# ChunLI-666/PointCloudProcessor

Hardware: AMD Instinct MI355X
Metric: Mpoints×frames/sec colorized (higher is better)
Workload: dtype f32/f64

## Files before the change

### include/pcp_hip.h

```cpp
#ifndef PCP_HIP_H
#define PCP_HIP_H

#include <stdint.h>

#ifdef __cplusplus
extern "C" {
#endif

#define PCP_ABI_VERSION 6

#define PCP_OK 0
#define PCP_ERR_INVALID (-1)
#define PCP_ERR_STATE (-2)
#define PCP_ERR_DEVICE (-3)
#define PCP_ERR_NOMEM (-4)
#define PCP_ERR_RANGE (-5)

typedef struct pcp_context pcp_context;

typedef struct pcp_pose {
  double x, y, z, qw, qx, qy, qz;
} pcp_pose;

typedef struct pcp_camera {
// ... 202 lines not shown
#define PCP_ASCII_PARSE_MAX_ROW 65536
#define PCP_PARSE_LIMIT_ROW 0
#define PCP_PARSE_LIMIT_TILE 1
#define PCP_PARSE_LIMIT_PIECE 2
#define PCP_PARSE_LIMIT_TILE_ROWS 3
#define PCP_PARSE_LIMIT_WINDOW 4
int64_t pcp_ascii_parse_limit(int32_t which);
int pcp_ascii_parse_host(const char *text, int64_t bytes, int32_t columns, const int32_t col[4], int32_t final_window,
                         int64_t max_rows, float *out_x, float *out_y, float *out_z, float *out_intensity,
                         int64_t *out_rows, int64_t *out_consumed, int64_t *out_bad_row);
int pcp_ascii_parse(pcp_context *ctx, const char *text, int64_t bytes, int32_t columns, const int32_t col[4], int32_t final_window,
                    int64_t max_rows, float *out_x, float *out_y, float *out_z, float *out_intensity,
                    int64_t *out_rows, int64_t *out_consumed, int64_t *out_bad_row);

int pcp_voxel_reduce_begin(pcp_context *ctx, float leaf, int64_t initial_slots);
int pcp_voxel_reduce_add(pcp_context *ctx, int64_t *out_rows_added);
int pcp_voxel_reduce_finish(pcp_context *ctx, int64_t *out_voxels);
int pcp_voxel_reduce_fetch(pcp_context *ctx, int64_t first, int64_t max_rows, float *out_xyz, uint8_t *out_rgb, uint8_t *out_label,
                           uint32_t *out_count, int64_t *out_rows);
int pcp_voxel_reduce_stats(pcp_context *ctx, int64_t out[6]);
int pcp_voxel_reduce_end(pcp_context *ctx);
int pcp_voxel_reduce_host(float leaf, int64_t n, const float *xyz, const uint8_t *rgb, const uint8_t *label, int64_t capacity,
                          float *out_xyz, uint8_t *out_rgb, uint8_t *out_label, uint32_t *out_count, int64_t *out_voxels);

typedef struct pcp_ortho_frame {
  float o[3], u[3], v[3], n[3];
  float gsd;
  int32_t width, height;
  float d_min, d_max;
} pcp_ortho_frame;
int pcp_ortho_begin(pcp_context *ctx, const pcp_ortho_frame *frame);
int pcp_ortho_add(pcp_context *ctx, int64_t index_base, int64_t *out_contributors);
int pcp_ortho_add_packed(pcp_context *ctx, const uint32_t *rgba, int64_t index_base, int64_t *out_contributors);
int pcp_ortho_finish(pcp_context *ctx, int32_t fill_radius_px, int64_t *out_occupied, int64_t *out_filled);
int pcp_ortho_fetch(pcp_context *ctx, uint32_t *out_index, float *out_depth, uint8_t *out_rgb, uint8_t *out_label,
                    uint8_t *out_status, int32_t *out_source);
int pcp_ortho_stats(pcp_context *ctx, int64_t out[6]);
int pcp_ortho_end(pcp_context *ctx);
int pcp_ortho_host(const pcp_ortho_frame *frame, int64_t n, const float *xyz, const uint8_t *rgb, const uint8_t *label,
                   const uint8_t *has, int64_t index_base, int32_t fill_radius_px, uint32_t *out_index, float *out_depth,
                   uint8_t *out_rgb, uint8_t *out_label, uint8_t *out_status, int32_t *out_source, int64_t *out_contributors,
                   int64_t *out_occupied, int64_t *out_filled);
int pcp_ortho_fit_frame_host(int64_t n, const float *xyz, const uint8_t *has, const double *viewer, float gsd, pcp_ortho_frame *out);

typedef struct pcp_ortho_texture_params {
  int32_t scale;
  int32_t x0, y0, w, h;
  int32_t views;
  int32_t interpolate;
  float max_step;
} pcp_ortho_texture_params;
int pcp_ortho_texture(pcp_context *ctx, const pcp_ortho_texture_params *params, uint8_t *out_rgb, uint8_t *out_mask,
                      uint8_t *out_status, int16_t *out_view, uint8_t *out_count, int64_t out_counts[4]);
int pcp_ortho_texture_points_host(const pcp_ortho_frame *frame, const pcp_ortho_texture_params *params, const int32_t *source,
                                  const float *depth, float *out_xyz, uint8_t *out_ok);

#define PCP_BALANCE_CLAHE 1
#define PCP_BALANCE_GAMMA 2
typedef struct pcp_balance_params {
  int32_t stages;
  int32_t tiles_x, tiles_y;
  float clip_limit;
  float gamma;
} pcp_balance_params;
void pcp_default_balance_params(pcp_balance_params *p);
int pcp_set_image_balance(pcp_context *ctx, const pcp_balance_params *params);
int pcp_image_balance_host(const pcp_balance_params *params, int32_t w, int32_t h, const uint8_t *bgr, int64_t row_stride_bytes,
                           uint8_t *out_bgr, uint32_t *out_hist, uint8_t *out_lut);
int pcp_image_balance(pcp_context *ctx, const pcp_balance_params *params, int32_t w, int32_t h, const uint8_t *bgr,
                      int64_t row_stride_bytes, uint8_t *out_bgr, uint32_t *out_hist, uint8_t *out_lut);
int pcp_gamma_table_host(float gamma, uint8_t out[256]);

int pcp_estimate_normals(pcp_context *ctx, float radius, int64_t *out_valid, int64_t *out_moments);
int pcp_normals_fetch(pcp_context *ctx, float *out_normal, float *out_curvature, int32_t *out_neighbours);
int pcp_normals_moments_host(float radius, int64_t n, const float *xyz, int64_t *out_moments);
int pcp_frame_geometry(pcp_context *ctx, int32_t frame, int32_t *out_index, float *out_range, float *out_xyz_cam,
                       float *out_normal_cam, int64_t *out_pixels);

int pcp_mask_edt(pcp_context *ctx, int32_t frame, int32_t threshold, uint32_t *out_d2, int32_t *out_nearest);
int pcp_mask_edt_frames(pcp_context *ctx, int32_t first_frame, int32_t count, int32_t threshold, uint32_t *out_d2,
                        int32_t *out_nearest);
int pcp_mask_edt_host(int32_t width, int32_t height, const uint8_t *gray, int64_t row_stride_bytes, int32_t threshold,
                      uint32_t *out_d2, int32_t *out_nearest);

typedef struct pcp_crack_params {
  int32_t threshold;
  int32_t plane_radius_px;
} pcp_crack_params;
int pcp_crack_width(pcp_context *ctx, int32_t frame, const pcp_crack_params *params, uint8_t *out_flags, int32_t *out_edges,
                    uint32_t *out_w2d2, float *out_width, float *out_points, float *out_plane, int64_t *out_moments,
                    int64_t *out_sites, int64_t *out_widths);
int pcp_crack_width_host(int32_t width, int32_t height, const uint8_t *gray, int64_t row_stride_bytes, const int32_t *index_image,
                         const float *xyz_cam_image, const pcp_crack_params *params, uint8_t *out_flags, int32_t *out_edges,
                         uint32_t *out_w2d2, int64_t *out_moments);

typedef struct pcp_crack_link_params {
  int32_t min_views;
  float radius;
} pcp_crack_link_params;
int pcp_crack_fuse_begin(pcp_context *ctx);
int pcp_crack_fuse_add(pcp_context *ctx, int32_t frame, const pcp_crack_params *params, int64_t *out_contributors,
                       int64_t *out_credited);
int pcp_crack_fuse_fetch(pcp_context *ctx, float *out_width_mean, float *out_width_best, int32_t *out_best_frame, uint32_t *out_views,
                         uint32_t *out_seen, uint32_t *out_centres, uint32_t *out_min_q, uint32_t *out_max_q, uint64_t *out_sum_q);
int pcp_crack_fuse_end(pcp_context *ctx);
int pcp_crack_fuse_host(int64_t n, uint32_t *seen, uint32_t *views, uint32_t *centres, uint32_t *min_q, uint32_t *max_q,
                        uint32_t *best_q, uint64_t *sum_q, uint64_t *best_key, int64_t m, const int32_t *index, const int32_t *pixel,
                        const float *range, int32_t frame, int32_t width, int32_t height, const uint8_t *flags, const float *width_image,
                        int64_t *out_credited);
int pcp_crack_components(pcp_context *ctx, const pcp_crack_link_params *p, int32_t *out_label, int64_t *out_crack_points,
                         int64_t *out_components);
int pcp_crack_components_fetch(pcp_context *ctx, int64_t first, int64_t max_rows, int32_t *out_id, int64_t *out_stats, float *out_box,
                               int64_t *out_rows);
int pcp_crack_components_host(int64_t n, const float *xyz, const uint32_t *views, int32_t min_views, float radius, int32_t *out_label,
                              int64_t *out_components);

int pcp_crack_lengths(pcp_context *ctx, const pcp_crack_link_params *p, uint64_t *out_pos, int64_t *out_cracks, int64_t *out_path_points);
int pcp_crack_lengths_fetch(pcp_context *ctx, int64_t first, int64_t max_rows, int32_t *out_id, int64_t *out_rows7, int64_t *out_offsets,
                            int64_t *out_rows);
int pcp_crack_paths_fetch(pcp_context *ctx, int64_t first_entry, int64_t max_entries, int32_t *out_index, int64_t *out_entries);
int pcp_crack_lengths_host(int64_t n, const float *xyz, const uint32_t *views, int32_t min_views, float radius, const uint64_t *sum_q,
                           uint64_t *out_pos, int32_t *out_id, int64_t *out_rows7, int64_t *out_offsets, int32_t *out_path,
                           int64_t *out_cracks, int64_t *out_path_points);

int pcp_crack_skeleton(pcp_context *ctx, const pcp_crack_link_params *p, float step, int32_t *out_node, int64_t *out_nodes, int64_t *out_edges);
int pcp_crack_skeleton_nodes_fetch(pcp_context *ctx, int64_t first, int64_t max_rows, int32_t *out_id, int64_t *out_rows10, int64_t *out_rows);
int pcp_crack_skeleton_edges_fetch(pcp_context *ctx, int64_t first, int64_t max_rows, int64_t *out_rows3, int64_t *out_rows);
int pcp_crack_skeleton_cracks_fetch(pcp_context *ctx, int64_t first, int64_t max_rows, int64_t *out_rows6, int64_t *out_rows);
int pcp_crack_skeleton_host(int64_t n, const float *xyz, const uint32_t *views, int32_t min_views, float radius, float step,
                            const uint64_t *sum_q, int32_t *out_node, int32_t *out_id, int64_t *out_rows10, int64_t edge_capacity,
                            int64_t *out_rows3, int64_t *out_rows6, int64_t *out_nodes, int64_t *out_edges, int64_t *out_cracks);

typedef struct pcp_facet_params {
  float link_radius, angle_deg, plane_tol, max_curvature;
  int32_t min_points;
} pcp_facet_params;
int pcp_facets(pcp_context *ctx, const pcp_facet_params *params, int32_t *out_label, int64_t *out_facet_points, int64_t *out_components,
               int64_t *out_facets);
int pcp_facets_fetch(pcp_context *ctx, int64_t first, int64_t max_rows, int32_t *out_id, int64_t *out_rows10, float *out_box,
                     int64_t *out_rows);
int pcp_facets_host(int64_t n, const float *xyz, const float *normal, const float *curvature, const pcp_facet_params *params,
                    int32_t *out_label, int32_t *out_id, int64_t *out_rows10, float *out_box, int64_t *out_facets);
int pcp_facet_plane_host(const float root[3], const int64_t row10[10], double out_plane[7]);
int pcp_ortho_add_facet(pcp_context *ctx, int32_t facet_id, int64_t index_base, int64_t *out_contributors);

int pcp_close_pairs(pcp_context *ctx, double radius, int64_t *points_with_close_neighbour);

int pcp_timing_enable(pcp_context *ctx, int32_t on);
int pcp_timing_reset(pcp_context *ctx);
int pcp_timing_get(pcp_context *ctx, int32_t kernel_id, double *total_ms, int64_t *launches);
const char *pcp_kernel_name(int32_t kernel_id);
int pcp_tile_mask_density(pcp_context *ctx, double *kept_fraction);
int pcp_tile_masks(pcp_context *ctx, int64_t *tiles, int32_t *mask_words, uint32_t *out_words);
int pcp_sor_redo_fraction(pcp_context *ctx, double *fraction);
int pcp_sor_distances(pcp_context *ctx, int64_t capacity, float *out_distance);
int pcp_selftest_arithmetic(pcp_context *ctx, int64_t samples, uint64_t seed, int64_t *mismatches_fp64,
                            int64_t *mismatches_fp32);
int pcp_selftest_visit_forms(pcp_context *ctx, int64_t samples, uint64_t seed, int64_t *mismatches_uv, int64_t *mismatches_cell,
                             int64_t *mismatches_sqrt, int32_t *short_distortion);
int pcp_selftest_k3_term(pcp_context *ctx, int64_t samples, uint64_t seed, int64_t *mismatches, int32_t *term_dropped);

#ifdef __cplusplus
}
#endif
#endif
```

### pointcloudprocessor_amd/_build.py

```python
from __future__ import annotations

import os
import subprocess

_PKG = os.path.dirname(os.path.abspath(__file__))
_ROOT = os.path.dirname(_PKG)
CSRC = os.path.join(_PKG, "csrc")
LIB_DIR = os.path.join(_PKG, "lib")
LIB_PATH = os.path.join(LIB_DIR, "libpcp_hip.so")
INCLUDE = os.path.join(_ROOT, "include")

SOURCES = ["pcp_context.hip", "pcp_colour.hip", "pcp_mls.hip", "pcp_grid.hip", "pcp_nid.hip", "pcp_hpr.hip", "pcp_colour_smooth.hip", "pcp_match.hip", "pcp_jpeg.hip",
           "pcp_stream_colour.hip", "pcp_ascii.hip", "pcp_ascii_parse.hip", "pcp_exposure.hip", "pcp_voxel_reduce.hip", "pcp_normals.hip", "pcp_mask_edt.hip", "pcp_ortho.hip", "pcp_ortho_texture.hip", "pcp_facets.hip", "pcp_crack_width.hip", "pcp_crack_fuse.hip", "pcp_crack_length.hip", "pcp_crack_skeleton.hip", "pcp_image_balance.hip"]
HEADERS = ["pcp_internal.hpp", "pcp_device.hpp", "pcp_scan.hpp", "pcp_hsv.hpp", "pcp_exact.hpp", "pcp_ascii.hpp", "pcp_ascii_parse.hpp", "pcp_visit_forms.hpp", "pcp_voxel_reduce.hpp", "pcp_eigen33.hpp", "pcp_eigen33_host.hpp", "pcp_facets.hpp", "pcp_normals.hpp", "pcp_mask_edt.hpp", "pcp_ortho.hpp", "pcp_ortho_texture.hpp", "pcp_tile_classify.hpp", "pcp_crack_width.hpp", "pcp_crack_fuse.hpp", "pcp_crack_length.hpp", "pcp_crack_skeleton.hpp", "pcp_crack_map.hpp", "pcp_image_balance.hpp"]

HIPCC_FLAGS = [
    "--offload-arch=gfx950",
    "-O3",
    "-std=c++17",
    "-fPIC",
    "-ffp-contract=off",
    "-fhip-fp32-correctly-rounded-divide-sqrt",
    "-Wall",
    "-Wextra",
]


def _hipcc() -> str:
    for cand in (os.environ.get("HIPCC"), "/opt/rocm/bin/hipcc", "hipcc"):
        if cand and (os.path.isabs(cand) and os.path.exists(cand) or not os.path.isabs(cand)):
            return cand
    return "hipcc"


def source_sha256() -> str:
    import hashlib

    h = hashlib.sha256()
    h.update(" ".join(HIPCC_FLAGS).encode())
    for f in [os.path.join(CSRC, f) for f in SOURCES + HEADERS] + [os.path.join(INCLUDE, "pcp_hip.h")]:
        h.update(os.path.basename(f).encode())
        with open(f, "rb") as fh:
            h.update(fh.read())
    return h.hexdigest()


def is_stale() -> bool:
    if not os.path.exists(LIB_PATH):
        return True
    t = os.path.getmtime(LIB_PATH)
    deps = [os.path.join(CSRC, f) for f in SOURCES + HEADERS] + [os.path.join(INCLUDE, "pcp_hip.h")]
    return any(os.path.getmtime(d) > t for d in deps)


def build(force: bool = False, verbose: bool = False) -> str:
    if not force and not is_stale():
        return LIB_PATH
    os.makedirs(LIB_DIR, exist_ok=True)
    from concurrent.futures import ThreadPoolExecutor

    obj_dir = os.path.join(LIB_DIR, "obj")
    os.makedirs(obj_dir, exist_ok=True)
    inc = ["-I", os.path.relpath(INCLUDE, CSRC), "-I", "."]

    def compile_one(src):
        stem = os.path.splitext(src)[0]
        obj = os.path.join(os.path.relpath(obj_dir, CSRC), stem + ".o")
        cmd = [_hipcc()] + HIPCC_FLAGS + inc + [f"-cuid={stem}", "-c", src, "-o", obj]
        return cmd, subprocess.run(cmd, capture_output=True, text=True, cwd=CSRC)

    with ThreadPoolExecutor(max_workers=len(SOURCES)) as pool:
        results = list(pool.map(compile_one, SOURCES))
    log = ""
    for cmd, proc in results:
        if verbose or proc.returncode != 0:
            log += " ".join(cmd) + "\n" + proc.stdout + proc.stderr
    if any(proc.returncode != 0 for _, proc in results):
        print(log)
        raise RuntimeError("hipcc failed building libpcp_hip.so:\n" + log[-4000:])
    objs = [os.path.join(os.path.relpath(obj_dir, CSRC), os.path.splitext(src)[0] + ".o") for src in SOURCES]
    link = [_hipcc(), "--offload-arch=gfx950", "--hip-link", "-shared", "-fPIC", "-o", LIB_PATH] + objs
    proc = subprocess.run(link, capture_output=True, text=True, cwd=CSRC)
    if verbose or proc.returncode != 0:
        print(log + " ".join(link))
        print(proc.stdout)
        print(proc.stderr)
    if proc.returncode != 0:
        raise RuntimeError("hipcc failed linking libpcp_hip.so:\n" + proc.stderr[-4000:])
    return LIB_PATH


if __name__ == "__main__":
    print(build(force=True, verbose=True))
```

### pointcloudprocessor_amd/capi.py

```python
from __future__ import annotations

import ctypes as C
import os
import re

import numpy as np

from . import _build

PCP_OK = 0
PCP_ERR_INVALID = -1
PCP_ERR_STATE = -2
PCP_ERR_DEVICE = -3
PCP_ERR_NOMEM = -4
PCP_ERR_RANGE = -5

NID_EVAL_FN = C.CFUNCTYPE(C.c_int, C.c_void_p, C.POINTER(C.c_double), C.c_int32, C.POINTER(C.c_double), C.POINTER(C.c_double),
                          C.POINTER(C.c_int32))
K_PROJECT, K_DEPTH, K_COLOUR, K_VISIBILITY, K_MLS_GRID, K_MLS_FIT, K_MISC, K_SOR, K_MLS_VOXEL, K_TILE_MASK, K_NID, K_HPR = range(12)
K_COLOUR_SMOOTH = 12
K_COUNT = 13


class PcpError(RuntimeError):
# ... 1394 lines not shown
    def sor(self, mean_k: int = 60, std_mul: float = 0.7):
        keep = np.empty(self.n, np.uint8)
        kept = C.c_int64()
        self._check(self.lib.pcp_sor(self.h, C.c_int32(mean_k), C.c_double(std_mul), _ptr(keep), C.byref(kept)))
        return keep, kept.value

    def sor_chunk_points(self) -> int:
        return int(self.lib.pcp_sor_chunk_points())

    def sor_partial(self, mean_k: int, slab: int, n_slabs: int):
        c = self.sor_chunk_points()
        chunks = (self.n + c - 1) // c
        out = np.zeros((max(chunks, 1), 2), np.float64)
        first, cnt = C.c_int64(), C.c_int64()
        self._check(self.lib.pcp_sor_partial(self.h, C.c_int32(mean_k), C.c_int32(slab), C.c_int32(n_slabs), C.c_int64(len(out)),
                                             _ptr(out), C.byref(first), C.byref(cnt)))
        return first.value, out[:cnt.value].copy()

    def sor_finish(self, std_mul: float, all_chunk_sums: np.ndarray, slab: int, n_slabs: int):
        sums = np.ascontiguousarray(all_chunk_sums, np.float64)
        keep = np.empty(self.n, np.uint8)
        kept = C.c_int64()
        self._check(self.lib.pcp_sor_finish(self.h, C.c_double(std_mul), _ptr(sums), C.c_int64(len(sums)), C.c_int32(slab),
                                            C.c_int32(n_slabs), _ptr(keep), C.byref(kept)))
        return keep, kept.value

    def close_pairs(self, radius: float = 2.5e-5) -> int:
        cnt = C.c_int64()
        self._check(self.lib.pcp_close_pairs(self.h, C.c_double(radius), C.byref(cnt)))
        return cnt.value

    def sor_distances(self) -> np.ndarray:
        out = np.empty(self.n, np.float32)
        self._check(self.lib.pcp_sor_distances(self.h, C.c_int64(len(out)), _ptr(out)))
        return out

    def sor_redo_fraction(self) -> float:
        v = C.c_double()
        self._check(self.lib.pcp_sor_redo_fraction(self.h, C.byref(v)))
        return v.value

    def upload_intensity(self, intensity):
        a = np.ascontiguousarray(intensity, np.float32)
        self._check(self.lib.pcp_upload_intensity(self.h, _ptr(a), C.c_int64(len(a))))

    def nid_prepare(self) -> int:
        cnt = C.c_int64()
        self._check(self.lib.pcp_nid_prepare(self.h, C.byref(cnt)))
        return cnt.value

    def nid_evaluate(self, T, T_init=None, bins: int = 16):
        T = np.ascontiguousarray(T, np.float64).reshape(16)
        Ti = None if T_init is None else np.ascontiguousarray(T_init, np.float64).reshape(16)
        cost = C.c_double()
        grad = np.zeros(6, np.float64)
        valid = C.c_int32()
        self._check(self.lib.pcp_nid_evaluate(self.h, _ptr(T), _ptr(Ti), C.c_int32(bins), C.byref(cost), _ptr(grad),
                                              C.byref(valid)))
        return cost.value, grad, bool(valid.value)

    def nid_optimize(self, T_init, bins: int = 16, max_outer_iterations: int = 10):
        Ti = np.ascontiguousarray(T_init, np.float64).reshape(16)
        out = np.zeros(16, np.float64)
        cost = C.c_double()
        evals = C.c_int32()
        self._check(self.lib.pcp_nid_optimize(self.h, _ptr(Ti), C.c_int32(bins), C.c_int32(max_outer_iterations), _ptr(out),
                                              C.byref(cost), C.byref(evals)))
        return out.reshape(4, 4), cost.value, evals.value

    def nid_accumulate(self, T, bins: int = 16):
        T = np.ascontiguousarray(T, np.float64).reshape(16)
        self._check(self.lib.pcp_nid_accumulate(self.h, _ptr(T), C.c_int32(bins)))

    def nid_histograms_device(self):
        p = C.c_void_p()
        n = C.c_int64()
        self._check(self.lib.pcp_nid_histograms_device(self.h, C.byref(p), C.byref(n)))
        return p.value, n.value

    def nid_finish(self, bins: int = 16):
        cost = C.c_double()
        grad = np.zeros(6, np.float64)
        valid = C.c_int32()
        self._check(self.lib.pcp_nid_finish(self.h, C.c_int32(bins), C.byref(cost), _ptr(grad), C.byref(valid)))
        return cost.value, grad, bool(valid.value)

    def nid_optimize_with(self, evaluate, T_init, bins: int = 16, max_outer_iterations: int = 10):
        errors = []

        @NID_EVAL_FN
        def trampoline(_user, T, b, cost, grad, valid):
            try:
                c, g, ok = evaluate(np.ctypeslib.as_array(T, (16,)).copy().reshape(4, 4), int(b))
                cost[0] = float(c)
                for k in range(6):
                    grad[k] = float(g[k])
                valid[0] = 1 if ok else 0
                return 0
            except Exception as e:
                errors.append(e)
                return -3

        Ti = np.ascontiguousarray(T_init, np.float64).reshape(16)
        out = np.zeros(16, np.float64)
        cost = C.c_double()
        evals = C.c_int32()
        rc = self.lib.pcp_nid_optimize_with(self.h, trampoline, None, _ptr(Ti), C.c_int32(bins), C.c_int32(max_outer_iterations),
                                            _ptr(out), C.byref(cost), C.byref(evals))
        if errors:
            raise errors[0]
        self._check(rc)
        return out.reshape(4, 4), cost.value, evals.value

    def timing_enable(self, on: bool = True):
        self._check(self.lib.pcp_timing_enable(self.h, C.c_int32(1 if on else 0)))

    def timing_reset(self):
        self._check(self.lib.pcp_timing_reset(self.h))

    def timing_get(self, kernel_id: int):
        ms = C.c_double()
        cnt = C.c_int64()
        self._check(self.lib.pcp_timing_get(self.h, C.c_int32(kernel_id), C.byref(ms), C.byref(cnt)))
        return ms.value, cnt.value

    def tile_mask_density(self) -> float:
        v = C.c_double()
        self._check(self.lib.pcp_tile_mask_density(self.h, C.byref(v)))
        return v.value

    def selftest_arithmetic(self, samples: int = 1 << 26, seed: int = 1):
        a, b = C.c_int64(), C.c_int64()
        self._check(self.lib.pcp_selftest_arithmetic(self.h, C.c_int64(samples), C.c_uint64(seed), C.byref(a), C.byref(b)))
        return a.value, b.value

    def selftest_visit_forms(self, samples: int = 1 << 24, seed: int = 1):
        a, b, c, f = C.c_int64(), C.c_int64(), C.c_int64(), C.c_int32()
        self._check(self.lib.pcp_selftest_visit_forms(self.h, C.c_int64(samples), C.c_uint64(seed), C.byref(a), C.byref(b), C.byref(c),
                                                      C.byref(f)))
        return a.value, b.value, c.value, bool(f.value)

    def selftest_k3_term(self, samples: int = 1 << 24, seed: int = 1):
        a, f = C.c_int64(), C.c_int32()
        self._check(self.lib.pcp_selftest_k3_term(self.h, C.c_int64(samples), C.c_uint64(seed), C.byref(a), C.byref(f)))
        return a.value, bool(f.value)

    def tile_masks(self) -> np.ndarray:
        t, w = C.c_int64(), C.c_int32()
        self._check(self.lib.pcp_tile_masks(self.h, C.byref(t), C.byref(w), None))
        out = np.empty((t.value, w.value), np.uint32)
        self._check(self.lib.pcp_tile_masks(self.h, None, None, _ptr(out)))
        return out

    def kernel_name(self, kernel_id: int) -> str:
        return self.lib.pcp_kernel_name(C.c_int32(kernel_id)).decode()
```

### pointcloudprocessor_amd/csrc/pcp_colour.hip

```cpp
#include <algorithm>
#include <cfloat>
#include <cstdlib>

#include "pcp_device.hpp"
#include "pcp_hsv.hpp"
#include "pcp_scan.hpp"
#include "pcp_tile_classify.hpp"

namespace pcp {

constexpr int kBlock = 256;
constexpr uint32_t kFltMaxBits = 0x7f7fffffu;

template <bool kCommon>
__device__ __forceinline__ DevCamera common_camera(const DevCamera &in) {
  DevCamera c = in;
  if constexpr (kCommon) {
    c.cull_mode = PCP_CULL_ZBUFFER;
    c.enable_zbuf = 1;
    c.pretest = 1;
    c.ds_fast = 1;
  }
  return c;
}
inline bool is_common_camera(const pcp_context *ctx) {
  const DevCamera &c = ctx->dcam;
  return c.cull_mode == PCP_CULL_ZBUFFER && c.enable_zbuf == 1 && c.pretest == 1 && c.ds_fast == 1 && ctx->uv_tame;
}

struct ProjectOut {
  int32_t *cell;
  int32_t *pixel;
  float *range;
  float *xc, *yc, *zc;
};

__device__ __forceinline__ void project_store_one(const DevCamera &cam, const DevFrame &fr, float x, float y, float z,
                                                  int32_t &cell, int32_t &pixel, float &range, float &xc, float &yc,
                                                  float &zc) {
  const Projected p = project_point<true, false>(cam, fr.w2c, x, y, z);
  cell = p.cell;
  pixel = p.pixel;
  range = p.cell != -1 ? static_cast<float>(range64(p.xc, p.yc, p.zc)) : FLT_MAX;
  xc = p.xc;
  yc = p.yc;
  zc = p.zc;
}

template <bool kCommon>
__global__ __launch_bounds__(kBlock) void k_project_frame(const float *__restrict__ x, const float *__restrict__ y,
                                                          const float *__restrict__ z, int64_t n, DevCamera cam_in,
                                                          DevFrame fr, ProjectOut out) {
  const DevCamera cam = common_camera<kCommon>(cam_in);
  const int64_t q = static_cast<int64_t>(blockIdx.x) * kBlock + threadIdx.x;
  const int64_t i0 = q * 4;
  if (i0 >= n) return;
  if (i0 + 3 < n) {
    typedef float nt_f4 __attribute__((ext_vector_type(4)));
    typedef int nt_i4 __attribute__((ext_vector_type(4)));
    const nt_f4 ax = __builtin_nontemporal_load(reinterpret_cast<const nt_f4 *>(x + i0));
    const nt_f4 ay = __builtin_nontemporal_load(reinterpret_cast<const nt_f4 *>(y + i0));
    const nt_f4 az = __builtin_nontemporal_load(reinterpret_cast<const nt_f4 *>(z + i0));
    const float4 vx = make_float4(ax.x, ax.y, ax.z, ax.w), vy = make_float4(ay.x, ay.y, ay.z, ay.w),
                 vz = make_float4(az.x, az.y, az.z, az.w);
    int4 cell, pixel;
    float4 range, xc, yc, zc;
    project_store_one(cam, fr, vx.x, vy.x, vz.x, cell.x, pixel.x, range.x, xc.x, yc.x, zc.x);
    project_store_one(cam, fr, vx.y, vy.y, vz.y, cell.y, pixel.y, range.y, xc.y, yc.y, zc.y);
    project_store_one(cam, fr, vx.z, vy.z, vz.z, cell.z, pixel.z, range.z, xc.z, yc.z, zc.z);
    project_store_one(cam, fr, vx.w, vy.w, vz.w, cell.w, pixel.w, range.w, xc.w, yc.w, zc.w);
    if (out.cell) {
      const nt_i4 c4 = {cell.x, cell.y, cell.z, cell.w};
      __builtin_nontemporal_store(c4, reinterpret_cast<nt_i4 *>(out.cell + i0));
    }
    if (out.range) {
      const nt_f4 r4 = {range.x, range.y, range.z, range.w};
      __builtin_nontemporal_store(r4, reinterpret_cast<nt_f4 *>(out.range + i0));
    }
    if (out.pixel) *reinterpret_cast<int4 *>(out.pixel + i0) = pixel;
    if (out.xc) {
      *reinterpret_cast<float4 *>(out.xc + i0) = xc;
      *reinterpret_cast<float4 *>(out.yc + i0) = yc;
      *reinterpret_cast<float4 *>(out.zc + i0) = zc;
    }
  } else {
    for (int64_t i = i0; i < n; ++i) {
      int32_t cell, pixel;
      float range, xc, yc, zc;
      project_store_one(cam, fr, x[i], y[i], z[i], cell, pixel, range, xc, yc, zc);
      if (out.cell) out.cell[i] = cell;
      if (out.range) out.range[i] = range;
      if (out.pixel) out.pixel[i] = pixel;
      if (out.xc) {
        out.xc[i] = xc;
        out.yc[i] = yc;
        out.zc[i] = zc;
      }
    }
  }
}

constexpr int kTileGroup = 16;

__global__ __launch_bounds__(kBlock) void k_group_mask_flat(const float4 *__restrict__ spheres, int64_t groups, DevCamera cam,
                                                            const DevFrame *__restrict__ frames, int32_t n_frames,
                                                            int32_t w0, int32_t w1, int32_t words,
                                                            uint32_t *__restrict__ group_mask,
                                                            uint32_t *__restrict__ group_inside, int32_t cull_enabled,
                                                            int32_t *__restrict__ zeroed, int32_t n_zeroed,
                                                            unsigned long long *__restrict__ far_maps, int64_t far_cells) {
  const int64_t idx = static_cast<int64_t>(blockIdx.x) * kBlock + threadIdx.x;
  if (idx < n_zeroed) zeroed[idx] = 0;
  for (int64_t c = idx; c < far_cells; c += static_cast<int64_t>(gridDim.x) * kBlock) far_maps[c] = 0x7f7f7f7f7f7f7f7full;
  const int32_t nw = w1 - w0;
  const int64_t gw = idx >> 5;
  const int64_t group = gw / nw;
  const bool live = group < groups;
  const int32_t w = w0 + static_cast<int32_t>(gw - group * nw);
  const int32_t f = (w << 5) + static_cast<int32_t>(idx & 31);
  int cls = 1;
  if (live && f < n_frames) cls = cull_enabled ? tile_classify(cam, frames[f], spheres[group]) : 0;
  const unsigned long long m = __ballot(cls != 1), in = __ballot(cls == 2);
  if (live && (idx & 31) == 0) {
    group_mask[group * words + w] = static_cast<uint32_t>((threadIdx.x & 32) ? (m >> 32) : m);
    group_inside[group * words + w] = static_cast<uint32_t>((threadIdx.x & 32) ? (in >> 32) : in);
  }
}

template <bool kInside>
__global__ __launch_bounds__(kBlock) void k_tile_mask_dense(const float4 *__restrict__ spheres, int64_t tiles,
                                                            DevCamera cam, const DevFrame *__restrict__ frames,
                                                            int32_t n_frames, int32_t w0, int32_t w1, int32_t words,
                                                            const uint32_t *__restrict__ group_mask,
                                                            const uint32_t *__restrict__ group_inside,
                                                            uint32_t *__restrict__ tile_mask,
                                                            uint32_t *__restrict__ inside_mask, int32_t cull_enabled) {
  const int lane = threadIdx.x & 63;
  const int32_t nw = w1 - w0;
  const int64_t gw = static_cast<int64_t>(blockIdx.x) * (kBlock / 64) + (threadIdx.x >> 6);
  const int64_t group = gw / nw;
  if (group >= (tiles + kTileGroup - 1) / kTileGroup) return;
  const int32_t w = w0 + static_cast<int32_t>(gw - group * nw);
  const int t = lane & 15, slot = lane >> 4;
  const int64_t tile = group * kTileGroup + t;
  const bool have = tile < tiles;
  uint32_t todo = __builtin_amdgcn_readfirstlane(group_mask[group * words + w]);
  const int32_t nb = n_frames - (w << 5);
  if (nb < 32) todo &= nb <= 0 ? 0u : ((1u << nb) - 1u);
  const uint32_t whole = __builtin_amdgcn_readfirstlane(group_inside[group * words + w]) & todo;
  todo &= ~whole;
  uint32_t word = whole;
  [[maybe_unused]] uint32_t inside = whole;
  if (todo) {
    const float4 sph = spheres[have ? tile : tiles - 1];
    while (todo) {
      int32_t bit[4];
#pragma unroll
      for (int k = 0; k < 4; ++k) {
        bit[k] = todo ? __builtin_ctz(todo) : -1;
        todo &= todo - (todo ? 1u : 0u);
      }
      const int32_t b = slot == 0 ? bit[0] : slot == 1 ? bit[1] : slot == 2 ? bit[2] : bit[3];
      int cls = 1;
      if (b >= 0 && have) cls = cull_enabled ? tile_classify(cam, frames[(w << 5) + b], sph) : 0;
      const unsigned long long keep = __ballot(cls != 1);
      [[maybe_unused]] unsigned long long ins = 0ull;
      if constexpr (kInside) ins = __ballot(cls == 2);
#pragma unroll
      for (int k = 0; k < 4; ++k) {
        if (bit[k] >= 0) {
          word |= static_cast<uint32_t>((keep >> (k * 16 + t)) & 1ull) << bit[k];
          if constexpr (kInside) inside |= static_cast<uint32_t>((ins >> (k * 16 + t)) & 1ull) << bit[k];
        }
      }
    }
  }
  if (slot == 0 && have) {
    tile_mask[tile * words + w] = word;
    if constexpr (kInside) {
      if (inside_mask) inside_mask[tile * words + w] = inside;
    }
  }
}

constexpr int kWorkBins = 1024;
constexpr int kWorkPerBlock = 1024;
__global__ __launch_bounds__(kBlock) void k_tile_work_hist(const uint32_t *__restrict__ tile_mask, int64_t tiles, int32_t w0,
                                                          int32_t w1, int32_t words, int32_t *__restrict__ tile_work,
                                                          int32_t *__restrict__ hist) {
  __shared__ int32_t cnt[kWorkBins];
  for (int b = threadIdx.x; b < kWorkBins; b += kBlock) cnt[b] = 0;
  __syncthreads();
  const int64_t base = static_cast<int64_t>(blockIdx.x) * kWorkPerBlock;
  for (int q = 0; q < kWorkPerBlock / kBlock; ++q) {
    const int64_t t = base + q * kBlock + threadIdx.x;
    if (t < tiles) {
      int32_t visits = 0;
      for (int32_t w = w0; w < w1; ++w) visits += __builtin_popcount(tile_mask[t * words + w]);
      tile_work[t] = visits;
      atomicAdd(&cnt[min(visits, kWorkBins - 1)], 1);
    }
  }
  __syncthreads();
  for (int b = threadIdx.x; b < kWorkBins; b += kBlock)
    if (cnt[b]) atomicAdd(&hist[b], cnt[b]);
}
__global__ __launch_bounds__(kBlock) void k_work_scatter(const int32_t *__restrict__ work, int64_t tiles,
                                                        const int32_t *__restrict__ hist, int32_t *__restrict__ cursor,
                                                        int32_t *__restrict__ order) {
  __shared__ int32_t cnt[kWorkBins];
  __shared__ int32_t first[kWorkBins];
  __shared__ int32_t ws[kScanBlock / 64];
  for (int b = threadIdx.x; b < kWorkBins; b += kBlock) cnt[b] = 0;
  {
    constexpr int kPer = kWorkBins / kBlock;
    int32_t h[kPer], mine = 0;
#pragma unroll
    for (int k = 0; k < kPer; ++k) {
      h[k] = hist[kWorkBins - 1 - (static_cast<int>(threadIdx.x) * kPer + k)];
      mine += h[k];
    }
    int32_t total = 0;
    int32_t run = scan_block_exclusive(mine, &total, ws);
#pragma unroll
    for (int k = 0; k < kPer; ++k) {
      first[kWorkBins - 1 - (static_cast<int>(threadIdx.x) * kPer + k)] = run;
      run += h[k];
    }
  }
  __syncthreads();
  const int64_t base = static_cast<int64_t>(blockIdx.x) * kWorkPerBlock;
  int32_t bin[kWorkPerBlock / kBlock], rank[kWorkPerBlock / kBlock];
#pragma unroll
  for (int q = 0; q < kWorkPerBlock / kBlock; ++q) {
    const int64_t t = base + q * kBlock + threadIdx.x;
    bin[q] = t < tiles ? min(work[t], kWorkBins - 1) : -1;
    rank[q] = bin[q] >= 0 ? atomicAdd(&cnt[bin[q]], 1) : 0;
  }
  __syncthreads();
  for (int b = threadIdx.x; b < kWorkBins; b += kBlock)
    if (cnt[b]) cnt[b] = first[b] + atomicAdd(&cursor[b], cnt[b]);
  __syncthreads();
#pragma unroll
  for (int q = 0; q < kWorkPerBlock / kBlock; ++q)
    if (bin[q] >= 0) order[cnt[bin[q]] + rank[q]] = static_cast<int32_t>(base + q * kBlock + threadIdx.x);
}

constexpr uint32_t kXcdChunk = 16;
__device__ __forceinline__ uint32_t xcd_chunked_block() {
  constexpr uint32_t kXcd = 8, kSuper = kXcd * kXcdChunk;
  const uint32_t b = blockIdx.x;
  if (b >= (gridDim.x / kSuper) * kSuper) return b;
  const uint32_t x = b % kXcd, slot = b / kXcd;
  return ((slot / kXcdChunk) * kXcd + x) * kXcdChunk + slot % kXcdChunk;
}

constexpr unsigned long long kDepthEmpty = 0x7f7f7f7f7f7f7f7full;
__device__ __forceinline__ void depth_min(unsigned long long *__restrict__ map, int32_t cell, unsigned long long bits) {
  if (bits < map[cell]) atomicMin(map + cell, bits);
}
__device__ __forceinline__ double sumsq64(float xc, float yc, float zc) {
  const double X = xc, Y = yc, Z = zc;
  return (X * X + Y * Y) + Z * Z;
}
__global__ __launch_bounds__(kBlock) void k_depth_finish(const unsigned long long *__restrict__ sq, int64_t count,
                                                         uint32_t *__restrict__ range) {
  int64_t i = static_cast<int64_t>(blockIdx.x) * kBlock + threadIdx.x;
  const int64_t stride = static_cast<int64_t>(gridDim.x) * kBlock;
  for (; i < count; i += stride) {
    const unsigned long long b = sq[i];
    float r = FLT_MAX;
    if (b != kDepthEmpty) r = fminf(static_cast<float>(sqrt(__longlong_as_double(static_cast<long long>(b)))), FLT_MAX);
    range[i] = __float_as_uint(r);
  }
}

__device__ __forceinline__ uint32_t range_bits(int32_t w, int32_t f0, int32_t f1) {
  const int32_t fb = max(f0, w << 5), fe = min(f1, (w << 5) + 32);
  const int32_t nb = fe - fb;
  return nb <= 0 ? 0u : (((nb >= 32) ? 0xffffffffu : ((1u << nb) - 1u)) << (fb & 31));
}

template <bool kCommon, bool kK3 = true>
__global__ __launch_bounds__(kBlock) void k_depth_pass(const float *__restrict__ x, const float *__restrict__ y,
                                                       const float *__restrict__ z, int64_t n, DevCamera cam_in,
                                                       const DevFrame *__restrict__ frames, int32_t f0, int32_t f1,
                                                       unsigned long long *__restrict__ depth, int64_t cells,
                                                       int32_t depth_first_frame, uint32_t *__restrict__ tile_mask,
                                                       const uint32_t *__restrict__ tile_inside, int32_t words,
                                                       const int32_t *__restrict__ tile_order) {
  DevCamera cam = common_camera<kCommon>(cam_in);
  if constexpr (kCommon) cam.pretest = 0;
  __shared__ unsigned long long combine[kBlock];
  const int lane = threadIdx.x & 63;
  unsigned long long *tbl = combine + (threadIdx.x & ~63);
  const int64_t j = tile_order ? static_cast<int64_t>(tile_order[blockIdx.x]) * 64 + threadIdx.x
                               : static_cast<int64_t>(xcd_chunked_block()) * kBlock + threadIdx.x;
  const bool live = j < n;
  if (!__ballot(live)) return;
  const float px = live ? x[j] : 0.0f, py = live ? y[j] : 0.0f, pz = live ? z[j] : 0.0f;
  const int64_t tile = __builtin_amdgcn_readfirstlane(static_cast<int32_t>(j >> 6));
  const bool finite_sure = cam.frames_bounded != 0 && __all(fabsf(px) <= 0x1p40f && fabsf(py) <= 0x1p40f && fabsf(pz) <= 0x1p40f);
  unsigned long long *held_at = nullptr;
  unsigned long long held_bits = 0ull, held_seen = 0ull;
  auto settle_held = [&]() {
    if (held_at && held_bits < held_seen) atomicMin(held_at, held_bits);
    held_at = nullptr;
  };
  const int32_t w_last = (f1 - 1) >> 5;
  for (int32_t wbase = f0 >> 5; wbase <= w_last; wbase += 64) {
    const int32_t my_w = wbase + lane;
    const bool have_w = my_w <= w_last;
    uint32_t my_word = 0xffffffffu;
    if (tile_mask && have_w) my_word = tile_mask[tile * words + my_w];
    [[maybe_unused]] uint32_t my_inside = 0u;
    if constexpr (!kCommon) {
      if (tile_inside && have_w) my_inside = tile_inside[tile * words + my_w];
// ... 1277 lines not shown

int pcp_project_frame(pcp_context *ctx, int32_t frame, int32_t *out_cell, int32_t *out_pixel, float *out_range,
                      float *out_xyz_cam) {
  int rc = check_ready(ctx, "pcp_project_frame", true);
  if (rc != PCP_OK) return rc;
  if ((rc = check_frame(ctx, "pcp_project_frame", frame)) != PCP_OK) return rc;
  const int64_t n = ctx->n;
  const size_t plane = plane_of(ctx);
  PCP_HIP_TRY(ctx, ctx->s_cell.ensure(plane + 4));
  PCP_HIP_TRY(ctx, ctx->s_range.ensure(plane + 4));
  if (out_pixel) PCP_HIP_TRY(ctx, ctx->s_pixel.ensure(plane + 4));
  if (out_xyz_cam) PCP_HIP_TRY(ctx, ctx->s_cam.ensure(3 * plane + 4));
  if (n == 0) return PCP_OK;
  ProjectOut o{};
  o.cell = ctx->s_cell.p;
  o.range = ctx->s_range.p;
  o.pixel = out_pixel ? ctx->s_pixel.p : nullptr;
  o.xc = out_xyz_cam ? ctx->s_cam.p : nullptr;
  o.yc = out_xyz_cam ? ctx->s_cam.p + plane : nullptr;
  o.zc = out_xyz_cam ? ctx->s_cam.p + 2 * plane : nullptr;
  {
    LaunchTimer t(ctx, PCP_K_PROJECT);
    hipLaunchKernelGGL(is_common_camera(ctx) ? k_project_frame<true> : k_project_frame<false>, dim3(blocks_for(div_up(n, 4))), dim3(kBlock), 0, ctx->stream, ctx->sxyz.p,
                       ctx->sxyz.p + plane, ctx->sxyz.p + 2 * plane, n, ctx->dcam,
                       ctx->hframes[static_cast<size_t>(frame)], o);
    PCP_HIP_TRY(ctx, hipGetLastError());
  }
  if (!(out_cell || out_range || out_pixel || out_xyz_cam)) return PCP_OK;
  const size_t sn = static_cast<size_t>(n);
  PCP_HIP_TRY(ctx, ctx->s_u32.ensure(plane + 4));
  auto fetch = [&](const void *sorted, void *host) -> int {
    {
      LaunchTimer t(ctx, PCP_K_MISC);
      hipLaunchKernelGGL(k_scatter_u32, dim3(blocks_for(n)), dim3(kBlock), 0, ctx->stream,
                         static_cast<const uint32_t *>(sorted), ctx->perm.p, n, ctx->s_u32.p);
      PCP_HIP_TRY(ctx, hipGetLastError());
    }
    PCP_HIP_TRY(ctx, hipMemcpyAsync(host, ctx->s_u32.p, sn * 4, hipMemcpyDeviceToHost, ctx->stream));
    PCP_HIP_TRY(ctx, hipStreamSynchronize(ctx->stream));
    return PCP_OK;
  };
  if (out_cell && (rc = fetch(o.cell, out_cell)) != PCP_OK) return rc;
  if (out_range && (rc = fetch(o.range, out_range)) != PCP_OK) return rc;
  if (out_pixel && (rc = fetch(o.pixel, out_pixel)) != PCP_OK) return rc;
  if (out_xyz_cam) {
    if ((rc = fetch(o.xc, out_xyz_cam)) != PCP_OK) return rc;
    if ((rc = fetch(o.yc, out_xyz_cam + sn)) != PCP_OK) return rc;
    if ((rc = fetch(o.zc, out_xyz_cam + 2 * sn)) != PCP_OK) return rc;
  }
  return PCP_OK;
}

int pcp_cull_frame(pcp_context *ctx, int32_t frame, uint8_t *out_keep, int64_t *out_kept, float *out_depth_map) {
  int rc = check_ready(ctx, "pcp_cull_frame", true);
  if (rc != PCP_OK) return rc;
  if ((rc = check_frame(ctx, "pcp_cull_frame", frame)) != PCP_OK) return rc;
  const int64_t n = ctx->n;
  if ((rc = single_frame_depth(ctx, frame)) != PCP_OK) return rc;
  if ((rc = frame_keep_flags(ctx, frame, false)) != PCP_OK) return rc;
  if (out_kept) {
    int64_t cnt = 0;
    if (n > 0 && (rc = compact_flags(ctx, ctx->s_keep.p, n, nullptr, 0, &cnt)) != PCP_OK) return rc;
    *out_kept = cnt;
  }
  if (out_keep && n > 0)
    PCP_HIP_TRY(ctx, hipMemcpyAsync(out_keep, ctx->s_keep.p, static_cast<size_t>(n), hipMemcpyDefault, ctx->stream));
  if (out_depth_map)
    PCP_HIP_TRY(ctx, hipMemcpyAsync(out_depth_map, ctx->s_u32.p, static_cast<size_t>(cells_of(ctx)) * 4,
                                    hipMemcpyDeviceToHost, ctx->stream));
  PCP_HIP_TRY(ctx, hipStreamSynchronize(ctx->stream));
  return PCP_OK;
}

int pcp_frame_visible(pcp_context *ctx, int32_t frame, int64_t capacity, int32_t *out_index, uint8_t *out_rgb,
                      uint16_t *out_mask, float *out_xyz_cam, float *out_xyz_world, int64_t *out_count) {
  int rc = check_ready(ctx, "pcp_frame_visible", true);
  if (rc != PCP_OK) return rc;
  if ((rc = check_frame(ctx, "pcp_frame_visible", frame)) != PCP_OK) return rc;
  if (capacity < 0) return set_error(ctx, PCP_ERR_INVALID, "pcp_frame_visible: negative capacity");
  const int64_t n = ctx->n;
  if (out_count) *out_count = 0;
  if (n == 0) return PCP_OK;
  if ((rc = ensure_images(ctx)) != PCP_OK) return rc;
  if ((rc = wait_images(ctx, frame, frame + 1)) != PCP_OK) return rc;
  int64_t m = 0;
  if ((rc = visible_indices(ctx, frame, &m)) != PCP_OK) return rc;
  const size_t plane = plane_of(ctx);
  if (out_count) *out_count = m;
  const int64_t take = std::min(m, capacity);
  if (take == 0) return PCP_OK;
  const size_t st = static_cast<size_t>(take);
  PCP_HIP_TRY(ctx, ctx->s_range.ensure(st + 4));
  const bool want_cam = out_xyz_cam != nullptr, want_world = out_xyz_world != nullptr;
  PCP_HIP_TRY(ctx, ctx->s_cam.ensure((want_cam ? 3 * st : 0) + (want_world ? 3 * st : 0) + 4));
  float *d_cam = want_cam ? ctx->s_cam.p : nullptr;
  float *d_world = want_world ? ctx->s_cam.p + (want_cam ? 3 * st : 0) : nullptr;
  const int64_t px = static_cast<int64_t>(ctx->dcam.img_w) * ctx->dcam.img_h;
  {
    LaunchTimer t(ctx, PCP_K_MISC);
    hipLaunchKernelGGL(k_gather_visible, dim3(blocks_for(take)), dim3(kBlock), 0, ctx->stream, ctx->xyz.p,
                       ctx->xyz.p + plane, ctx->xyz.p + 2 * plane, ctx->dcam, ctx->hframes[static_cast<size_t>(frame)],
                       ctx->s_cell.p, take, ctx->images.p + static_cast<int64_t>(frame) * px,
                       static_cast<int32_t>(ctx->image_set[static_cast<size_t>(frame)]),
                       static_cast<int32_t>(ctx->mask_set[static_cast<size_t>(frame)]),
                       reinterpret_cast<uint32_t *>(ctx->s_range.p), d_cam, d_world);
    PCP_HIP_TRY(ctx, hipGetLastError());
  }
  std::vector<uint32_t> rgbm;
  if (out_rgb || out_mask) {
    rgbm.resize(st);
    PCP_HIP_TRY(ctx, hipMemcpyAsync(rgbm.data(), ctx->s_range.p, st * 4, hipMemcpyDeviceToHost, ctx->stream));
  }
  if (out_index) PCP_HIP_TRY(ctx, hipMemcpyAsync(out_index, ctx->s_cell.p, st * 4, hipMemcpyDeviceToHost, ctx->stream));
  if (want_cam) PCP_HIP_TRY(ctx, hipMemcpyAsync(out_xyz_cam, d_cam, 3 * st * 4, hipMemcpyDeviceToHost, ctx->stream));
  if (want_world) PCP_HIP_TRY(ctx, hipMemcpyAsync(out_xyz_world, d_world, 3 * st * 4, hipMemcpyDeviceToHost, ctx->stream));
  PCP_HIP_TRY(ctx, hipStreamSynchronize(ctx->stream));
  for (size_t k = 0; k < rgbm.size(); ++k) {
    if (out_rgb) {
      out_rgb[3 * k + 0] = static_cast<uint8_t>(rgbm[k] & 0xffu);
      out_rgb[3 * k + 1] = static_cast<uint8_t>((rgbm[k] >> 8) & 0xffu);
      out_rgb[3 * k + 2] = static_cast<uint8_t>((rgbm[k] >> 16) & 0xffu);
    }
    if (out_mask) out_mask[k] = static_cast<uint16_t>(rgbm[k] >> 24);
  }
  return PCP_OK;
}

int pcp_depth_pass(pcp_context *ctx, int32_t frame_begin, int32_t frame_end) {
  int rc = check_ready(ctx, "pcp_depth_pass", true);
  if (rc != PCP_OK) return rc;
  if (frame_begin < 0 || frame_end > ctx->n_frames || frame_begin > frame_end)
    return set_error(ctx, PCP_ERR_RANGE, "pcp_depth_pass: keyframe range [%d,%d) outside 0..%d", frame_begin, frame_end,
                     ctx->n_frames);
  if (frame_begin == frame_end) return PCP_OK;
  if ((rc = ensure_depth(ctx)) != PCP_OK) return rc;
  const int64_t cells = cells_of(ctx);
  const int64_t map_cells = static_cast<int64_t>(frame_end - frame_begin) * cells;
  const bool z_maps = ctx->n > 0 && ctx->dcam.enable_zbuf;
  if (z_maps) {
    PCP_HIP_TRY(ctx, ctx->depth_sq.ensure(static_cast<size_t>(map_cells) + 4));
  } else if ((rc = fill_u32(ctx, ctx->depth.p + static_cast<int64_t>(frame_begin) * cells, map_cells, kFltMaxBits)) != PCP_OK) {
    return rc;
  }
  if (ctx->n > 0) {
    const size_t plane = plane_of(ctx);
    const int32_t w0 = frame_begin >> 5, w1 = ((frame_end - 1) >> 5) + 1;
    static const bool cull_tiles = [] {
      const char *e = std::getenv("PCP_DISABLE_TILE_CULL");
      return !(e && e[0] == '1');
    }();
    {
      LaunchTimer t(ctx, PCP_K_TILE_MASK);
      const int64_t groups = div_up(ctx->n_tiles, kTileGroup);
      const float4 *tile_sph = reinterpret_cast<const float4 *>(ctx->tile_sphere.p);
      const size_t gwords = static_cast<size_t>(groups) * ctx->mask_words;
      PCP_HIP_TRY(ctx, ctx->group_mask.ensure(2 * gwords + 8));
      uint32_t *group_inside = ctx->group_mask.p + gwords + 4;
      hipLaunchKernelGGL(k_group_mask_flat, dim3(std::max(blocks_for(groups * (w1 - w0) * 32), blocks_for(2 * kWorkBins))),
                         dim3(kBlock), 0, ctx->stream, tile_sph + ctx->n_tiles, groups, ctx->dcam, ctx->frames.p, ctx->n_frames,
                         w0, w1, ctx->mask_words, ctx->group_mask.p, group_inside, cull_tiles ? 1 : 0, ctx->work_hist.p,
                         2 * kWorkBins, z_maps ? reinterpret_cast<unsigned long long *>(ctx->depth_sq.p) : nullptr,
                         z_maps ? map_cells : int64_t(0));
      uint32_t *tile_inside = is_common_camera(ctx) ? nullptr : ctx->tile_inside.p;
      hipLaunchKernelGGL(tile_inside ? k_tile_mask_dense<true> : k_tile_mask_dense<false>, dim3(static_cast<uint32_t>(div_up(groups * (w1 - w0), kBlock / 64))), dim3(kBlock),
                         0, ctx->stream, tile_sph, ctx->n_tiles, ctx->dcam, ctx->frames.p, ctx->n_frames, w0, w1,
                         ctx->mask_words, ctx->group_mask.p, group_inside, ctx->tile_mask.p, tile_inside, cull_tiles ? 1 : 0);
      if ((rc = sort_tiles_by_work(ctx, w0, w1, ctx->tile_order.p)) != PCP_OK) return rc;
      ctx->tile_order_live = true;
    }
    if (ctx->cull.cull_mode == PCP_CULL_HPR) {
      int rch = ensure_hull_bits(ctx);
      if (rch != PCP_OK) return rch;
      if (!ctx->depth_from_batch) {
        int32_t clear_until = frame_begin;
        for (int32_t f = frame_begin; f < frame_end; ++f) {
          uint32_t *hull_plane = ctx->hull_bits.p + static_cast<size_t>(f >> 5) * static_cast<size_t>(ctx->n);
          if ((f & 31) == 0 && std::min(f + 32, ctx->n_frames) <= frame_end) {
            PCP_HIP_TRY(ctx, hipMemsetAsync(hull_plane, 0, static_cast<size_t>(ctx->n) * 4, ctx->stream));
            clear_until = std::min(f + 32, ctx->n_frames);
          }
          if (f >= clear_until) {
            LaunchTimer t(ctx, PCP_K_HPR);
            hipLaunchKernelGGL(k_hull_clear, dim3(blocks_for(ctx->n)), dim3(kBlock), 0, ctx->stream, hull_plane, ctx->n, 1u << (f & 31));
          }
        }
        PCP_HIP_TRY(ctx, hipGetLastError());
        const char *le = std::getenv("PCP_HPR_LANES");
        const int32_t lanes = le && le[0] >= '1' && le[0] <= '8' ? le[0] - '0' : 4;
        if ((rc = hpr_run_range(ctx, frame_begin, frame_end, lanes, ctx->tile_mask.p)) != PCP_OK) return rc;
        for (int32_t f = frame_begin; f < frame_end; ++f) ctx->hull_valid[static_cast<size_t>(f)] = 1;
      }
    }
    {
      LaunchTimer t(ctx, PCP_K_DEPTH);
      const bool common = is_common_camera(ctx);
      auto kernel = !common ? k_depth_pass<false> : ctx->k3_dropped ? k_depth_pass<true, false> : k_depth_pass<true>;
      hipLaunchKernelGGL(kernel,
                         dim3(static_cast<uint32_t>(ctx->n_tiles)), dim3(64), 0, ctx->stream, ctx->sxyz.p,
                         ctx->sxyz.p + plane, ctx->sxyz.p + 2 * plane, ctx->n, ctx->dcam, ctx->frames.p, frame_begin,
                         frame_end, ctx->depth_sq.p, cells, frame_begin, ctx->tile_mask.p,
                         common ? static_cast<const uint32_t *>(nullptr) : ctx->tile_inside.p, ctx->mask_words, ctx->tile_order.p);
      if (z_maps)
        hipLaunchKernelGGL(k_depth_finish, dim3(static_cast<uint32_t>(std::min<int64_t>(div_up(map_cells, kBlock), 4096))),
                           dim3(kBlock), 0, ctx->stream, ctx->depth_sq.p, map_cells,
                           ctx->depth.p + static_cast<int64_t>(frame_begin) * cells);
      PCP_HIP_TRY(ctx, hipGetLastError());
    }
  }
  for (int32_t f = frame_begin; f < frame_end; ++f) ctx->depth_valid[static_cast<size_t>(f)] = 1;
  return PCP_OK;
}

int pcp_depth_maps_device(pcp_context *ctx, void **device_ptr, int64_t *n_floats) {
  int rc = check_ready(ctx, "pcp_depth_maps_device", true);
  if (rc != PCP_OK) return rc;
  if (ctx->cull.cull_mode == PCP_CULL_HPR)
    return set_error(ctx, PCP_ERR_STATE, "pcp_depth_maps_device: PCP_CULL_HPR has no depth maps to merge across point shards "
                     "(the hull needs the whole map on one GPU)");
  if ((rc = ensure_depth(ctx)) != PCP_OK) return rc;
  if (device_ptr) *device_ptr = ctx->depth.p;
  if (n_floats) *n_floats = cells_of(ctx) * ctx->n_frames;
  return PCP_OK;
}

int pcp_set_depth_source(pcp_context *ctx, int32_t source) {
  if (!ctx) return PCP_ERR_INVALID;
  if (source != PCP_DEPTH_OWN && source != PCP_DEPTH_BATCHED)
    return set_error(ctx, PCP_ERR_INVALID, "pcp_set_depth_source: unknown source %d", source);
  ctx->depth_from_batch = source == PCP_DEPTH_BATCHED;
  return PCP_OK;
}

int pcp_hull_flags_import(pcp_context *ctx, int32_t frame, const uint8_t *keep) {
  int rc = check_ready(ctx, "pcp_hull_flags_import", true);
  if (rc != PCP_OK) return rc;
  if ((rc = check_frame(ctx, "pcp_hull_flags_import", frame)) != PCP_OK) return rc;
  if (ctx->cull.cull_mode != PCP_CULL_HPR || !ctx->depth_from_batch)
    return set_error(ctx, PCP_ERR_STATE, "pcp_hull_flags_import: needs cull_mode PCP_CULL_HPR and pcp_set_depth_source(PCP_DEPTH_BATCHED)");
  if (!keep && ctx->n > 0) return set_error(ctx, PCP_ERR_INVALID, "pcp_hull_flags_import: NULL flags");
  if ((rc = ensure_hull_bits(ctx)) != PCP_OK) return rc;
  if (ctx->n > 0) {
    PCP_HIP_TRY(ctx, ctx->s_keep.ensure(static_cast<size_t>(ctx->n) + 16));
    PCP_HIP_TRY(ctx, hipMemcpyAsync(ctx->s_keep.p, keep, static_cast<size_t>(ctx->n), hipMemcpyDefault, ctx->stream));
    if ((rc = store_hull_bits(ctx, frame, false)) != PCP_OK) return rc;
    PCP_HIP_TRY(ctx, hipStreamSynchronize(ctx->stream));
  }
  ctx->hull_valid[static_cast<size_t>(frame)] = 1;
  return PCP_OK;
}

int pcp_download_depth_map(pcp_context *ctx, int32_t frame, float *out_depth_map) {
  int rc = check_ready(ctx, "pcp_download_depth_map", true);
  if (rc != PCP_OK) return rc;
  if ((rc = check_frame(ctx, "pcp_download_depth_map", frame)) != PCP_OK) return rc;
  if (!out_depth_map) return set_error(ctx, PCP_ERR_INVALID, "pcp_download_depth_map: NULL output");
  if (!ctx->depth.p || !ctx->depth_valid[static_cast<size_t>(frame)])
    return set_error(ctx, PCP_ERR_STATE, "pcp_download_depth_map: pcp_depth_pass has not covered keyframe %d", frame);
  const int64_t cells = cells_of(ctx);
  PCP_HIP_TRY(ctx, hipMemcpyAsync(out_depth_map, ctx->depth.p + static_cast<int64_t>(frame) * cells,
                                  static_cast<size_t>(cells) * 4, hipMemcpyDeviceToHost, ctx->stream));
  PCP_HIP_TRY(ctx, hipStreamSynchronize(ctx->stream));
  return PCP_OK;
}

int pcp_colour_reset(pcp_context *ctx) {
  if (!ctx) return PCP_ERR_INVALID;
  ctx->colour_state_live = false;
  ctx->colour_result_live = false;
  ctx->labels_live = false;
  return PCP_OK;
}

static int begin_result(pcp_context *ctx, uint32_t **dst) {
  const int32_t cur = ctx->rgba_cur ^ 1;
  PCP_HIP_TRY(ctx, ctx->rgba2[cur].ensure(static_cast<size_t>(ctx->n) + 4));
  if (ctx->copy_pending[cur]) {
    PCP_HIP_TRY(ctx, hipStreamWaitEvent(ctx->stream, ctx->copy_done[cur], 0));
    ctx->copy_pending[cur] = false;
  }
  *dst = ctx->rgba2[cur].p;
  return PCP_OK;
}

static int labels_begin(pcp_context *ctx) {
  ctx->labels_live = false;
  if (!ctx->label_fusion) return PCP_OK;
  PCP_HIP_TRY(ctx, ctx->labels.ensure(static_cast<size_t>(ctx->n) + 4));
  PCP_HIP_TRY(ctx, hipMemsetAsync(ctx->labels.p + ctx->n, 0, 4, ctx->stream));
  return PCP_OK;
}

static int labels_end(pcp_context *ctx) {
  if (!ctx->label_fusion) return PCP_OK;
  uint32_t bad = 0;
  uint32_t *dst = ctx->readback ? static_cast<uint32_t *>(ctx->readback) : &bad;
  PCP_HIP_TRY(ctx, hipMemcpyAsync(dst, ctx->labels.p + ctx->n, 4, hipMemcpyDeviceToHost, ctx->stream));
  PCP_HIP_TRY(ctx, hipStreamSynchronize(ctx->stream));
  if (*dst != 0)
    return set_error(ctx, PCP_ERR_RANGE, "label fusion: a view score outside [2^-3, 2) reached the label arithmetic "
                     "(final_score cannot produce one): no labels for this result");
  ctx->labels_live = true;
  return PCP_OK;
}

static int check_masks(pcp_context *ctx, int32_t frame_begin, int32_t frame_end) {
  if (!ctx->label_fusion) return PCP_OK;
  for (int32_t f = frame_begin; f < frame_end; ++f)
    if (static_cast<size_t>(f) >= ctx->mask_set.size() || !ctx->mask_set[static_cast<size_t>(f)])
      return set_error(ctx, PCP_ERR_STATE, "pcp_colour_pass: label fusion is on and no mask was uploaded for keyframe %d", f);
  return PCP_OK;
}

static int colour_pass_impl(pcp_context *ctx, int32_t frame_begin, int32_t frame_end, bool one_shot,
                            uint32_t *result = nullptr) {
  int rc = check_ready(ctx, "pcp_colour_pass", true);
  if (rc != PCP_OK) return rc;
  if (frame_begin < 0 || frame_end > ctx->n_frames || frame_begin > frame_end)
    return set_error(ctx, PCP_ERR_RANGE, "pcp_colour_pass: keyframe range [%d,%d) outside 0..%d", frame_begin, frame_end,
// ... 123 lines not shown
    if ((rc = finalise_gained(ctx, result)) != PCP_OK) return rc;
  } else if (n > 0) {
    TopState st{ctx->top_score.p, ctx->top_rgb.p, ctx->top_frame.p, ctx->view_count.p};
    LaunchTimer t(ctx, PCP_K_COLOUR);
    const bool label = ctx->label_fusion;
    const LabelOut lab{label ? ctx->labels.p : nullptr};
    if (label)
      hipLaunchKernelGGL(k_finalise_labels, dim3(blocks_for(n)), dim3(kBlock), 0, ctx->stream, n, st, ctx->perm.p, result, lab);
    else
      hipLaunchKernelGGL(k_finalise, dim3(blocks_for(n)), dim3(kBlock), 0, ctx->stream, n, st, ctx->perm.p, result);
    PCP_HIP_TRY(ctx, hipGetLastError());
  }
  if ((rc = labels_end(ctx)) != PCP_OK) return rc;
  if ((rc = end_result(ctx, out_rgb, out_has)) != PCP_OK) return rc;
  if ((out_count || out_top_score || out_top_rgb || out_top_frame) && n > 0) {
    std::vector<int32_t> perm(sn), cnt;
    std::vector<uint32_t> tmp(kTopM * sn);
    PCP_HIP_TRY(ctx, hipMemcpyAsync(perm.data(), ctx->perm.p, sn * 4, hipMemcpyDeviceToHost, ctx->stream));
    auto fetch5 = [&](const void *src, void *dst_v) -> int {
      PCP_HIP_TRY(ctx, hipMemcpyAsync(tmp.data(), src, kTopM * sn * 4, hipMemcpyDeviceToHost, ctx->stream));
      PCP_HIP_TRY(ctx, hipStreamSynchronize(ctx->stream));
      uint32_t *dst = static_cast<uint32_t *>(dst_v);
      for (size_t j = 0; j < sn; ++j)
        for (int k = 0; k < kTopM; ++k) dst[static_cast<size_t>(perm[j]) * kTopM + k] = tmp[static_cast<size_t>(k) * sn + j];
      return PCP_OK;
    };
    if (out_top_score && (rc = fetch5(ctx->top_score.p, out_top_score)) != PCP_OK) return rc;
    if (out_top_rgb && (rc = fetch5(ctx->top_rgb.p, out_top_rgb)) != PCP_OK) return rc;
    if (out_top_rgb && ctx->label_fusion)
      for (size_t k = 0; k < kTopM * sn; ++k) out_top_rgb[k] &= 0xffffffu;
    if (out_top_frame && (rc = fetch5(ctx->top_frame.p, out_top_frame)) != PCP_OK) return rc;
    if (out_count) {
      cnt.resize(sn);
      PCP_HIP_TRY(ctx, hipMemcpyAsync(cnt.data(), ctx->view_count.p, sn * 4, hipMemcpyDeviceToHost, ctx->stream));
      PCP_HIP_TRY(ctx, hipStreamSynchronize(ctx->stream));
      for (size_t j = 0; j < sn; ++j) out_count[perm[j]] = cnt[j];
    }
  }
  return PCP_OK;
}

static int refuse_gains(pcp_context *ctx, const char *who) {
  if (!ctx->gains_set) return PCP_OK;
  return set_error(ctx, PCP_ERR_STATE, "%s: exposure gains are set (pcp_set_frame_gains): they apply to pcp_colour_reset / "
                   "pcp_colour_pass / pcp_colour_finalise; clear them with pcp_set_frame_gains(NULL) for the one-shot call", who);
}

int pcp_colorize(pcp_context *ctx, uint8_t *out_rgb, uint8_t *out_has) {
  int rc = check_ready(ctx, "pcp_colorize", true);
  if (rc != PCP_OK) return rc;
  if ((rc = refuse_gains(ctx, "pcp_colorize")) != PCP_OK) return rc;
  if ((rc = check_masks(ctx, 0, ctx->n_frames)) != PCP_OK) return rc;
  pcp_colour_reset(ctx);
  if ((rc = pcp_depth_pass(ctx, 0, ctx->n_frames)) != PCP_OK) return rc;
  uint32_t *result = nullptr;
  if ((rc = begin_result(ctx, &result)) != PCP_OK) return rc;
  if ((rc = labels_begin(ctx)) != PCP_OK) return rc;
  if ((rc = colour_pass_impl(ctx, 0, ctx->n_frames, true, result)) != PCP_OK) return rc;
  if ((rc = labels_end(ctx)) != PCP_OK) return rc;
  return end_result(ctx, out_rgb, out_has);
}

int pcp_colorize_from_depth(pcp_context *ctx, uint8_t *out_rgb, uint8_t *out_has) {
  int rc = check_ready(ctx, "pcp_colorize_from_depth", true);
  if (rc != PCP_OK) return rc;
  if ((rc = refuse_gains(ctx, "pcp_colorize_from_depth")) != PCP_OK) return rc;
  pcp_colour_reset(ctx);
  uint32_t *result = nullptr;
  if ((rc = begin_result(ctx, &result)) != PCP_OK) return rc;
  if ((rc = labels_begin(ctx)) != PCP_OK) return rc;
  if ((rc = colour_pass_impl(ctx, 0, ctx->n_frames, true, result)) != PCP_OK) return rc;
  if ((rc = labels_end(ctx)) != PCP_OK) return rc;
  return end_result(ctx, out_rgb, out_has);
}

int pcp_colour_smooth_local(pcp_context *ctx, float radius, int64_t *out_has_count) {
  if (!ctx) return PCP_ERR_INVALID;
  if (!smooth_radius_ok(radius))
    return set_error(ctx, PCP_ERR_INVALID, "pcp_colour_smooth_local: radius %g outside (0, 1]", static_cast<double>(radius));
  if (!ctx->colour_result_live)
    return set_error(ctx, PCP_ERR_STATE, "pcp_colour_smooth_local: no result (call pcp_colorize / pcp_colour_finalise)");
  if (out_has_count) *out_has_count = 0;
  if (ctx->n == 0) return PCP_OK;
  PCP_HIP_TRY(ctx, hipSetDevice(ctx->device));
  const uint32_t *src = ctx->rgba2[ctx->rgba_cur].p;
  uint32_t *dst = nullptr;
  int rc = begin_result(ctx, &dst);
  if (rc != PCP_OK) return rc;
  if ((rc = colour_smooth_words(ctx, radius, src, dst, out_has_count)) != PCP_OK) return rc;
  return end_result(ctx, nullptr, nullptr);
}

int pcp_download_result_packed(pcp_context *ctx, uint32_t *out_rgba) {
  if (!ctx) return PCP_ERR_INVALID;
  if (!ctx->colour_result_live)
    return set_error(ctx, PCP_ERR_STATE, "pcp_download_result_packed: no result (call pcp_colorize / pcp_colour_finalise)");
  if (!out_rgba && ctx->n > 0) return set_error(ctx, PCP_ERR_INVALID, "pcp_download_result_packed: NULL output");
  if (ctx->n > 0)
    PCP_HIP_TRY(ctx, hipMemcpyAsync(out_rgba, ctx->rgba2[ctx->rgba_cur].p, static_cast<size_t>(ctx->n) * 4,
                                    hipMemcpyDeviceToHost, ctx->stream));
  PCP_HIP_TRY(ctx, hipStreamSynchronize(ctx->stream));
  return PCP_OK;
}

int pcp_download_result_packed_async(pcp_context *ctx, uint32_t *out_rgba) {
  if (!ctx) return PCP_ERR_INVALID;
  if (!ctx->colour_result_live)
    return set_error(ctx, PCP_ERR_STATE, "pcp_download_result_packed_async: no result (call pcp_colorize / pcp_colour_finalise)");
  if (!out_rgba && ctx->n > 0) return set_error(ctx, PCP_ERR_INVALID, "pcp_download_result_packed_async: NULL output");
  const int32_t cur = ctx->rgba_cur;
  PCP_HIP_TRY(ctx, hipStreamWaitEvent(ctx->copy_stream, ctx->result_ready[cur], 0));
  if (ctx->n > 0)
    PCP_HIP_TRY(ctx, hipMemcpyAsync(out_rgba, ctx->rgba2[cur].p, static_cast<size_t>(ctx->n) * 4, hipMemcpyDeviceToHost,
                                    ctx->copy_stream));
  PCP_HIP_TRY(ctx, hipEventRecord(ctx->copy_done[cur], ctx->copy_stream));
  ctx->copy_pending[cur] = true;
  return PCP_OK;
}

int pcp_download_wait_previous(pcp_context *ctx) {
  if (!ctx) return PCP_ERR_INVALID;
  const int32_t prev = ctx->rgba_cur ^ 1;
  if (ctx->copy_pending[prev]) PCP_HIP_TRY(ctx, hipEventSynchronize(ctx->copy_done[prev]));
  return PCP_OK;
}

int pcp_tile_mask_density(pcp_context *ctx, double *kept_fraction) {
  if (!ctx || !kept_fraction) return PCP_ERR_INVALID;
  if (!ctx->tile_mask.p || ctx->n_tiles == 0 || ctx->n_frames == 0)
    return set_error(ctx, PCP_ERR_STATE, "pcp_tile_mask_density: no masks (call pcp_depth_pass)");
  std::vector<uint32_t> h(static_cast<size_t>(ctx->n_tiles) * ctx->mask_words);
  PCP_HIP_TRY(ctx, hipMemcpyAsync(h.data(), ctx->tile_mask.p, h.size() * 4, hipMemcpyDeviceToHost, ctx->stream));
  PCP_HIP_TRY(ctx, hipStreamSynchronize(ctx->stream));
  uint64_t bits = 0;
  for (uint32_t w : h) bits += static_cast<uint64_t>(__builtin_popcount(w));
  *kept_fraction = static_cast<double>(bits) / (static_cast<double>(ctx->n_tiles) * ctx->n_frames);
  return PCP_OK;
}

int pcp_tile_masks(pcp_context *ctx, int64_t *tiles, int32_t *mask_words, uint32_t *out_words) {
  if (!ctx) return PCP_ERR_INVALID;
  if (!ctx->tile_mask.p || ctx->n_tiles == 0 || ctx->n_frames == 0)
    return set_error(ctx, PCP_ERR_STATE, "pcp_tile_masks: no masks (call pcp_depth_pass)");
  if (tiles) *tiles = ctx->n_tiles;
  if (mask_words) *mask_words = ctx->mask_words;
  if (out_words) {
    PCP_HIP_TRY(ctx, hipMemcpyAsync(out_words, ctx->tile_mask.p, static_cast<size_t>(ctx->n_tiles) * ctx->mask_words * 4,
                                    hipMemcpyDeviceToHost, ctx->stream));
    PCP_HIP_TRY(ctx, hipStreamSynchronize(ctx->stream));
  }
  return PCP_OK;
}

int pcp_colour_result_device(pcp_context *ctx, void **device_ptr, int64_t *n_words) {
  if (!ctx) return PCP_ERR_INVALID;
  if (!ctx->colour_result_live)
    return set_error(ctx, PCP_ERR_STATE, "pcp_colour_result_device: no result (call pcp_colorize / pcp_colour_finalise)");
  if (device_ptr) *device_ptr = ctx->rgba2[ctx->rgba_cur].p;
  if (n_words) *n_words = ctx->n;
  return PCP_OK;
}

int pcp_set_label_fusion(pcp_context *ctx, int32_t enable) {
  if (!ctx) return PCP_ERR_INVALID;
  const bool on = enable != 0;
  if (on != ctx->label_fusion && ctx->colour_state_live)
    return set_error(ctx, PCP_ERR_STATE, "pcp_set_label_fusion: a top-5 accumulation is live (its lists %s the masks): "
                     "call pcp_colour_reset first", ctx->label_fusion ? "hold" : "do not hold");
  ctx->label_fusion = on;
  return PCP_OK;
}

int pcp_colour_labels(pcp_context *ctx, uint8_t *out_label, uint8_t *out_hits, uint8_t *out_views) {
  if (!ctx) return PCP_ERR_INVALID;
  if (!ctx->labels_live)
    return set_error(ctx, PCP_ERR_STATE, "pcp_colour_labels: no labels (pcp_set_label_fusion(1), then pcp_colorize / "
                     "pcp_colorize_from_depth / pcp_colour_finalise)");
  const int64_t n = ctx->n;
  if (n == 0 || !(out_label || out_hits || out_views)) return PCP_OK;
  PCP_HIP_TRY(ctx, hipSetDevice(ctx->device));
  const size_t sn = static_cast<size_t>(n);
  PCP_HIP_TRY(ctx, ctx->s_keep.ensure(4 * sn + 16));
  uint8_t *d_label = ctx->s_keep.p, *d_hits = d_label + sn, *d_views = d_hits + sn;
  hipLaunchKernelGGL(k_unpack_labels, dim3(blocks_for(n)), dim3(kBlock), 0, ctx->stream, ctx->labels.p, n,
                     out_label ? d_label : nullptr, out_hits ? d_hits : nullptr, out_views ? d_views : nullptr);
  PCP_HIP_TRY(ctx, hipGetLastError());
  if (out_label) PCP_HIP_TRY(ctx, hipMemcpyAsync(out_label, d_label, sn, hipMemcpyDeviceToHost, ctx->stream));
  if (out_hits) PCP_HIP_TRY(ctx, hipMemcpyAsync(out_hits, d_hits, sn, hipMemcpyDeviceToHost, ctx->stream));
  if (out_views) PCP_HIP_TRY(ctx, hipMemcpyAsync(out_views, d_views, sn, hipMemcpyDeviceToHost, ctx->stream));
  PCP_HIP_TRY(ctx, hipStreamSynchronize(ctx->stream));
  return PCP_OK;
}

int pcp_colour_labels_device(pcp_context *ctx, void **device_ptr, int64_t *n_words) {
  if (!ctx) return PCP_ERR_INVALID;
  if (!ctx->labels_live)
    return set_error(ctx, PCP_ERR_STATE, "pcp_colour_labels_device: no labels (pcp_set_label_fusion(1), then pcp_colorize / "
                     "pcp_colorize_from_depth / pcp_colour_finalise)");
  if (device_ptr) *device_ptr = ctx->labels.p;
  if (n_words) *n_words = ctx->n;
  return PCP_OK;
}

int pcp_selftest_arithmetic(pcp_context *ctx, int64_t samples, uint64_t seed, int64_t *mismatches_fp64,
                            int64_t *mismatches_fp32) {
  if (!ctx) return PCP_ERR_INVALID;
  if (!ctx->have_camera) return set_error(ctx, PCP_ERR_STATE, "pcp_selftest_arithmetic: pcp_set_camera has not been called");
  PCP_HIP_TRY(ctx, hipSetDevice(ctx->device));
  if (samples < 0) return set_error(ctx, PCP_ERR_INVALID, "pcp_selftest_arithmetic: negative sample count");
  PCP_HIP_TRY(ctx, ctx->s_counter.ensure(4));
  unsigned long long *bad = ctx->s_counter.p;
  PCP_HIP_TRY(ctx, hipMemsetAsync(bad, 0, 16, ctx->stream));
  if (samples > 0)
    hipLaunchKernelGGL(k_selftest_div64, dim3(blocks_for(samples)), dim3(kBlock), 0, ctx->stream, samples, seed, bad);
  hipLaunchKernelGGL(k_selftest_div32, dim3((1u << 24) / kBlock), dim3(kBlock), 0, ctx->stream, ctx->dcam, bad + 1);
  PCP_HIP_TRY(ctx, hipGetLastError());
  unsigned long long h[2] = {0, 0};
  PCP_HIP_TRY(ctx, hipMemcpyAsync(h, bad, 16, hipMemcpyDeviceToHost, ctx->stream));
  PCP_HIP_TRY(ctx, hipStreamSynchronize(ctx->stream));
  if (mismatches_fp64) *mismatches_fp64 = static_cast<int64_t>(h[0]);
  if (mismatches_fp32) *mismatches_fp32 = static_cast<int64_t>(h[1]);
  return PCP_OK;
}

int pcp_selftest_visit_forms(pcp_context *ctx, int64_t samples, uint64_t seed, int64_t *mismatches_uv, int64_t *mismatches_cell,
                             int64_t *mismatches_sqrt, int32_t *short_distortion) {
  if (!ctx) return PCP_ERR_INVALID;
  if (!ctx->have_camera) return set_error(ctx, PCP_ERR_STATE, "pcp_selftest_visit_forms: pcp_set_camera has not been called");
  PCP_HIP_TRY(ctx, hipSetDevice(ctx->device));
  if (samples < 0) return set_error(ctx, PCP_ERR_INVALID, "pcp_selftest_visit_forms: negative sample count");
  PCP_HIP_TRY(ctx, ctx->s_counter.ensure(4));
  unsigned long long *bad = ctx->s_counter.p;
  PCP_HIP_TRY(ctx, hipMemsetAsync(bad, 0, 32, ctx->stream));
  if (samples > 0)
    hipLaunchKernelGGL(k_selftest_uv, dim3(blocks_for(samples)), dim3(kBlock), 0, ctx->stream, ctx->dcam, ctx->uv_tame ? 1 : 0, samples, seed, bad);
  hipLaunchKernelGGL(k_selftest_cell_sqrt, dim3((1u << 24) / kBlock), dim3(kBlock), 0, ctx->stream, ctx->dcam, bad + 1, bad + 2);
  PCP_HIP_TRY(ctx, hipGetLastError());
  unsigned long long h[3] = {0, 0, 0};
  PCP_HIP_TRY(ctx, hipMemcpyAsync(h, bad, 24, hipMemcpyDeviceToHost, ctx->stream));
  PCP_HIP_TRY(ctx, hipStreamSynchronize(ctx->stream));
  if (mismatches_uv) *mismatches_uv = static_cast<int64_t>(h[0]);
  if (mismatches_cell) *mismatches_cell = static_cast<int64_t>(h[1]);
  if (mismatches_sqrt) *mismatches_sqrt = static_cast<int64_t>(h[2]);
  if (short_distortion) *short_distortion = ctx->uv_tame ? 1 : 0;
  return PCP_OK;
}

int pcp_selftest_k3_term(pcp_context *ctx, int64_t samples, uint64_t seed, int64_t *mismatches, int32_t *term_dropped) {
  if (!ctx) return PCP_ERR_INVALID;
  if (!ctx->have_camera) return set_error(ctx, PCP_ERR_STATE, "pcp_selftest_k3_term: pcp_set_camera has not been called");
  PCP_HIP_TRY(ctx, hipSetDevice(ctx->device));
  if (samples < 0) return set_error(ctx, PCP_ERR_INVALID, "pcp_selftest_k3_term: negative sample count");
  PCP_HIP_TRY(ctx, ctx->s_counter.ensure(4));
  unsigned long long *bad = ctx->s_counter.p;
  PCP_HIP_TRY(ctx, hipMemsetAsync(bad, 0, 8, ctx->stream));
  hipLaunchKernelGGL(k_selftest_k3, dim3(blocks_for(samples + kK3Edges)), dim3(kBlock), 0, ctx->stream, ctx->dcam,
                     ctx->k3_dropped ? 2 : ctx->uv_tame ? 1 : 0, samples, seed, bad);
  PCP_HIP_TRY(ctx, hipGetLastError());
  unsigned long long h = 0;
  PCP_HIP_TRY(ctx, hipMemcpyAsync(&h, bad, 8, hipMemcpyDeviceToHost, ctx->stream));
  PCP_HIP_TRY(ctx, hipStreamSynchronize(ctx->stream));
  if (mismatches) *mismatches = static_cast<int64_t>(h);
  if (term_dropped) *term_dropped = ctx->k3_dropped ? 1 : 0;
  return PCP_OK;
}

}
```

### pointcloudprocessor_amd/csrc/pcp_context.hip

```cpp
#include <algorithm>
#include <cfloat>
#include <cmath>
#include <cstdlib>
#include <new>
#include <vector>

#include "pcp_internal.hpp"
#include "pcp_crack_map.hpp"
#include "pcp_visit_forms.hpp"
#include "pcp_scan.hpp"

namespace pcp {

static thread_local std::string g_error;

int set_error(const pcp_context *ctx, int code, const char *fmt, ...) {
  char buf[1024];
  va_list ap;
  va_start(ap, fmt);
  vsnprintf(buf, sizeof(buf), fmt, ap);
  va_end(ap);
  if (ctx)
    ctx->error = buf;
  else
// ... 122 lines not shown
  v = (v | (v << 2)) & 0x09249249u;
  return v;
}

__global__ __launch_bounds__(kUpBlock) void k_up_bbox(const float *__restrict__ x, const float *__restrict__ y,
                                                     const float *__restrict__ z, int64_t n,
                                                     float *__restrict__ partial ,
                                                     unsigned long long *__restrict__ nonfinite) {
  __shared__ float sh[6][kUpBlock / 64];
  float lo[3] = {FLT_MAX, FLT_MAX, FLT_MAX}, hi[3] = {-FLT_MAX, -FLT_MAX, -FLT_MAX};
  uint32_t bad = 0;
  for (int64_t i = static_cast<int64_t>(blockIdx.x) * kUpBlock + threadIdx.x; i < n; i += static_cast<int64_t>(gridDim.x) * kUpBlock) {
    const float v[3] = {x[i], y[i], z[i]};
    bool fin = true;
#pragma unroll
    for (int a = 0; a < 3; ++a) {
      const bool f = fabsf(v[a]) <= FLT_MAX;
      fin = fin && f;
      if (f && v[a] < lo[a]) lo[a] = v[a];
      if (f && v[a] > hi[a]) hi[a] = v[a];
    }
    bad += fin ? 0u : 1u;
  }
  {
    const unsigned long long any = __ballot(bad != 0);
    if (any) {
      for (int o = 32; o >= 1; o >>= 1) bad += __shfl_xor(bad, o, 64);
      if ((threadIdx.x & 63) == 0) atomicAdd(nonfinite, static_cast<unsigned long long>(bad));
    }
  }
#pragma unroll
  for (int a = 0; a < 3; ++a)
    for (int o = 32; o >= 1; o >>= 1) {
      lo[a] = fminf(lo[a], __shfl_xor(lo[a], o, 64));
      hi[a] = fmaxf(hi[a], __shfl_xor(hi[a], o, 64));
    }
  if ((threadIdx.x & 63) == 0)
    for (int a = 0; a < 3; ++a) {
      sh[a][threadIdx.x >> 6] = lo[a];
      sh[3 + a][threadIdx.x >> 6] = hi[a];
    }
  __syncthreads();
  if (threadIdx.x < 6) {
    float v = sh[threadIdx.x][0];
    for (int k = 1; k < kUpBlock / 64; ++k) v = threadIdx.x < 3 ? fminf(v, sh[threadIdx.x][k]) : fmaxf(v, sh[threadIdx.x][k]);
    partial[static_cast<int64_t>(blockIdx.x) * 6 + threadIdx.x] = v;
  }
}

__device__ __forceinline__ uint32_t hilbert30(uint32_t x, uint32_t y, uint32_t z) {
  uint32_t X[3] = {x, y, z};
  for (uint32_t Q = 512u; Q > 1u; Q >>= 1) {
    const uint32_t P = Q - 1u;
#pragma unroll
    for (int i = 0; i < 3; ++i) {
      if (X[i] & Q) {
        X[0] ^= P;
      } else {
        const uint32_t t = (X[0] ^ X[i]) & P;
        X[0] ^= t;
        X[i] ^= t;
      }
    }
  }
  X[1] ^= X[0];
  X[2] ^= X[1];
  uint32_t t = 0u;
  for (uint32_t Q = 512u; Q > 1u; Q >>= 1)
    if (X[2] & Q) t ^= Q - 1u;
  X[0] ^= t;
  X[1] ^= t;
  X[2] ^= t;
  return (spread10(X[0]) << 2) | (spread10(X[1]) << 1) | spread10(X[2]);
}

__global__ __launch_bounds__(kUpBlock) void k_up_keys(const float *__restrict__ x, const float *__restrict__ y,
                                                     const float *__restrict__ z, int64_t n, float mnx, float mny,
                                                     float mnz, float scx, float scy, float scz,
                                                     uint32_t *__restrict__ key, int32_t *__restrict__ val) {
  const int64_t i = static_cast<int64_t>(blockIdx.x) * kUpBlock + threadIdx.x;
  if (i >= n) return;
  const uint32_t ix = static_cast<uint32_t>(fminf(fmaxf((x[i] - mnx) * scx, 0.0f), 1023.0f));
  const uint32_t iy = static_cast<uint32_t>(fminf(fmaxf((y[i] - mny) * scy, 0.0f), 1023.0f));
  const uint32_t iz = static_cast<uint32_t>(fminf(fmaxf((z[i] - mnz) * scz, 0.0f), 1023.0f));
  key[i] = hilbert30(ix, iy, iz);
  val[i] = static_cast<int32_t>(i);
}

__global__ __launch_bounds__(kUpBlock) void k_up_radix_hist(const uint32_t *__restrict__ key, int64_t n, int32_t shift,
                                                           int32_t *__restrict__ hist, int64_t blocks) {
  __shared__ int32_t cnt[256];
  cnt[threadIdx.x] = 0;
  __syncthreads();
  const int64_t i = static_cast<int64_t>(blockIdx.x) * kUpBlock + threadIdx.x;
  if (i < n) atomicAdd(&cnt[(key[i] >> shift) & 0xffu], 1);
  __syncthreads();
  hist[static_cast<int64_t>(threadIdx.x) * blocks + blockIdx.x] = cnt[threadIdx.x];
}

__global__ __launch_bounds__(kUpBlock) void k_up_radix_scatter(const uint32_t *__restrict__ key_in,
                                                              const int32_t *__restrict__ val_in, int64_t n,
                                                              int32_t shift, const int32_t *__restrict__ offs,
                                                              int64_t blocks, uint32_t *__restrict__ key_out,
                                                              int32_t *__restrict__ val_out) {
  __shared__ int32_t wcount[kUpBlock / 64][256];
  __shared__ int32_t wbase[kUpBlock / 64][256];
  const int lane = threadIdx.x & 63, wave = threadIdx.x >> 6;
  for (int k = 0; k < kUpBlock / 64; ++k) wcount[k][threadIdx.x] = 0;
  __syncthreads();
  const int64_t i = static_cast<int64_t>(blockIdx.x) * kUpBlock + threadIdx.x;
  const bool valid = i < n;
  const uint32_t k = valid ? key_in[i] : 0u;
  const int32_t v = valid ? val_in[i] : 0;
  const uint32_t digit = (k >> shift) & 0xffu;
  unsigned long long peers = __ballot(valid);
#pragma unroll
  for (int b = 0; b < 8; ++b) {
    const bool bit = (digit >> b) & 1u;
    const unsigned long long m = __ballot(bit);
    peers &= bit ? m : ~m;
  }
  const int rank = __popcll(peers & ((1ull << lane) - 1ull));
  if (valid && rank == 0) wcount[wave][digit] = __popcll(peers);
  __syncthreads();
  {
    int32_t run = offs[static_cast<int64_t>(threadIdx.x) * blocks + blockIdx.x];
    for (int w = 0; w < kUpBlock / 64; ++w) {
      wbase[w][threadIdx.x] = run;
      run += wcount[w][threadIdx.x];
    }
  }
  __syncthreads();
  if (valid) {
    const int64_t pos = static_cast<int64_t>(wbase[wave][digit]) + rank;
    key_out[pos] = k;
    val_out[pos] = v;
  }
}

__global__ __launch_bounds__(kUpBlock) void k_up_gather(const float *__restrict__ x, const float *__restrict__ y,
                                                       const float *__restrict__ z, const int32_t *__restrict__ perm,
                                                       int64_t n, float *__restrict__ sx, float *__restrict__ sy,
                                                       float *__restrict__ sz, int32_t *__restrict__ inv_perm) {
  const int64_t j = static_cast<int64_t>(blockIdx.x) * kUpBlock + threadIdx.x;
  if (j >= n) return;
  const int32_t i = perm[j];
  sx[j] = x[i];
  sy[j] = y[i];
  sz[j] = z[i];
  if (inv_perm) inv_perm[i] = static_cast<int32_t>(j);
}

template <int kSpan>
__global__ __launch_bounds__(kUpBlock) void k_up_spheres(const float *__restrict__ sx, const float *__restrict__ sy,
                                                        const float *__restrict__ sz, int64_t n,
                                                        float4 *__restrict__ out, int64_t count) {
  constexpr int kLanes = kSpan >= kUpBlock ? kUpBlock : kSpan;
  constexpr int kPer = kSpan / kLanes;
  constexpr int kSpheresPerBlock = kUpBlock / kLanes;
  __shared__ double red[7][kUpBlock / 64];
  const int sub = threadIdx.x / kLanes, l = threadIdx.x % kLanes;
  const int64_t sphere = static_cast<int64_t>(blockIdx.x) * kSpheresPerBlock + sub;
  const int64_t b = sphere * kSpan;
  double lo[3] = {1e300, 1e300, 1e300}, hi[3] = {-1e300, -1e300, -1e300};
  float px[kPer], py[kPer], pz[kPer];
  bool have[kPer];
#pragma unroll
  for (int q = 0; q < kPer; ++q) {
    const int64_t j = b + static_cast<int64_t>(q) * kLanes + l;
    have[q] = sphere < count && j < n;
    px[q] = have[q] ? sx[j] : 0.0f;
    py[q] = have[q] ? sy[j] : 0.0f;
    pz[q] = have[q] ? sz[j] : 0.0f;
    if (have[q]) {
      lo[0] = fmin(lo[0], static_cast<double>(px[q])); hi[0] = fmax(hi[0], static_cast<double>(px[q]));
      lo[1] = fmin(lo[1], static_cast<double>(py[q])); hi[1] = fmax(hi[1], static_cast<double>(py[q]));
      lo[2] = fmin(lo[2], static_cast<double>(pz[q])); hi[2] = fmax(hi[2], static_cast<double>(pz[q]));
    }
  }
#pragma unroll
  for (int a = 0; a < 3; ++a)
    for (int o = (kLanes < 64 ? kLanes : 64) / 2; o >= 1; o >>= 1) {
      lo[a] = fmin(lo[a], __shfl_xor(lo[a], o, 64));
      hi[a] = fmax(hi[a], __shfl_xor(hi[a], o, 64));
    }
  if (kLanes > 64) {
    if ((threadIdx.x & 63) == 0)
      for (int a = 0; a < 3; ++a) {
        red[a][threadIdx.x >> 6] = lo[a];
        red[3 + a][threadIdx.x >> 6] = hi[a];
      }
    __syncthreads();
    for (int a = 0; a < 3; ++a)
      for (int k = 0; k < kUpBlock / 64; ++k) {
        lo[a] = fmin(lo[a], red[a][k]);
        hi[a] = fmax(hi[a], red[3 + a][k]);
      }
    __syncthreads();
  }
  float c[3];
#pragma unroll
  for (int a = 0; a < 3; ++a) c[a] = static_cast<float>(0.5 * (lo[a] + hi[a]));
  double r2 = 0.0;
#pragma unroll
  for (int q = 0; q < kPer; ++q)
    if (have[q]) {
      const double dx = static_cast<double>(px[q]) - static_cast<double>(c[0]);
      const double dy = static_cast<double>(py[q]) - static_cast<double>(c[1]);
      const double dz = static_cast<double>(pz[q]) - static_cast<double>(c[2]);
      r2 = fmax(r2, (dx * dx + dy * dy) + dz * dz);
    }
  for (int o = (kLanes < 64 ? kLanes : 64) / 2; o >= 1; o >>= 1) r2 = fmax(r2, __shfl_xor(r2, o, 64));
  if (kLanes > 64) {
    if ((threadIdx.x & 63) == 0) red[6][threadIdx.x >> 6] = r2;
    __syncthreads();
    for (int k = 0; k < kUpBlock / 64; ++k) r2 = fmax(r2, red[6][k]);
  }
  if (l == 0 && sphere < count) {
    float r = static_cast<float>(sqrt(r2) * (1.0 + 1e-6));
    r = isfinite(r) ? __uint_as_float(__float_as_uint(r) + 1u) : r;
    out[sphere] = make_float4(c[0], c[1], c[2], r);
  }
}

static inline uint32_t up_blocks(int64_t n) { return static_cast<uint32_t>(std::max<int64_t>(1, (n + kUpBlock - 1) / kUpBlock)); }

__global__ __launch_bounds__(kUpBlock) void k_up_deinterleave(const uint32_t *__restrict__ aos, int64_t stride_words,
                                                             int64_t n, float *__restrict__ x, float *__restrict__ y,
                                                             float *__restrict__ z) {
  const int64_t i = static_cast<int64_t>(blockIdx.x) * kUpBlock + threadIdx.x;
  if (i >= n) return;
  const uint32_t *p = aos + i * stride_words;
  x[i] = __uint_as_float(p[0]);
  y[i] = __uint_as_float(p[1]);
  z[i] = __uint_as_float(p[2]);
}

int spatial_order(pcp_context *ctx, const float *dx, const float *dy, const float *dz, int64_t n, int32_t *perm, float *sx,
                  float *sy, float *sz, int32_t *inv_perm, float mn[3], float mx[3], unsigned long long *out_nonfinite) {
  hipStream_t st = ctx->stream;
  const size_t sn = static_cast<size_t>(n);
  const uint32_t bb_blocks = std::min<uint32_t>(up_blocks(n), 1024u);
  DevBuf<float> partial;
  PCP_HIP_TRY(ctx, partial.ensure(static_cast<size_t>(bb_blocks) * 6));
  PCP_HIP_TRY(ctx, ctx->s_counter.ensure(4));
  PCP_HIP_TRY(ctx, hipMemsetAsync(ctx->s_counter.p, 0, 8, st));
  hipLaunchKernelGGL(k_up_bbox, dim3(bb_blocks), dim3(kUpBlock), 0, st, dx, dy, dz, n, partial.p, ctx->s_counter.p);
  std::vector<float> hp(static_cast<size_t>(bb_blocks) * 6);
  unsigned long long nonfinite = 0;
  PCP_HIP_TRY(ctx, hipMemcpyAsync(hp.data(), partial.p, hp.size() * 4, hipMemcpyDeviceToHost, st));
  PCP_HIP_TRY(ctx, hipMemcpyAsync(&nonfinite, ctx->s_counter.p, 8, hipMemcpyDeviceToHost, st));
  PCP_HIP_TRY(ctx, hipStreamSynchronize(st));
  if (out_nonfinite) *out_nonfinite = nonfinite;
  partial.release();
  for (int a = 0; a < 3; ++a) {
    mn[a] = FLT_MAX;
    mx[a] = -FLT_MAX;
  }
  for (uint32_t b = 0; b < bb_blocks; ++b)
    for (int a = 0; a < 3; ++a) {
      mn[a] = std::min(mn[a], hp[static_cast<size_t>(b) * 6 + a]);
      mx[a] = std::max(mx[a], hp[static_cast<size_t>(b) * 6 + 3 + a]);
    }
  float sc[3];
  for (int a = 0; a < 3; ++a) {
    if (mn[a] > mx[a]) mn[a] = mx[a] = 0.0f;
    const float ext = mx[a] - mn[a];
    sc[a] = (ext > 0.0f && ext < FLT_MAX) ? 1023.999f / ext : 0.0f;
  }
  const int64_t blocks = up_blocks(n);
  DevBuf<uint32_t> key_a, key_b;
  DevBuf<int32_t> val_b, hist;
  PCP_HIP_TRY(ctx, key_a.ensure(sn + 4));
  PCP_HIP_TRY(ctx, key_b.ensure(sn + 4));
  PCP_HIP_TRY(ctx, val_b.ensure(sn + 4));
  const int64_t hm = 256 * blocks;
  PCP_HIP_TRY(ctx, hist.ensure(static_cast<size_t>(hm) + 8));
  hipLaunchKernelGGL(k_up_keys, dim3(up_blocks(n)), dim3(kUpBlock), 0, st, dx, dy, dz, n, mn[0], mn[1], mn[2], sc[0], sc[1],
                     sc[2], key_a.p, perm);
  uint32_t *kin = key_a.p, *kout = key_b.p;
  int32_t *vin = perm, *vout = val_b.p;
  for (int pass = 0; pass < 4; ++pass) {
    const int32_t shift = 8 * pass;
    hipLaunchKernelGGL(k_up_radix_hist, dim3(static_cast<uint32_t>(blocks)), dim3(kUpBlock), 0, st, kin, n, shift, hist.p, blocks);
    PCP_HIP_TRY(ctx, hipMemsetAsync(hist.p + hm, 0, sizeof(int32_t), st));
    PCP_HIP_TRY(ctx, scan_exclusive(st, hist.p, hm + 1, ctx->s_tiles, nullptr));
    hipLaunchKernelGGL(k_up_radix_scatter, dim3(static_cast<uint32_t>(blocks)), dim3(kUpBlock), 0, st, kin, vin, n, shift,
                       hist.p, blocks, kout, vout);
    std::swap(kin, kout);
    std::swap(vin, vout);
  }
  PCP_HIP_TRY(ctx, hipGetLastError());
  hipLaunchKernelGGL(k_up_gather, dim3(up_blocks(n)), dim3(kUpBlock), 0, st, dx, dy, dz, perm, n, sx, sy, sz, inv_perm);
  PCP_HIP_TRY(ctx, hipGetLastError());
  PCP_HIP_TRY(ctx, hipStreamSynchronize(st));
  return PCP_OK;
}

static int store_cloud(pcp_context *ctx, const float *x, const float *y, const float *z, int64_t n,
                       const void *aos = nullptr, int64_t stride = 0, bool aos_on_device = false, bool copy_aside = false) {
  PCP_HIP_TRY(ctx, hipSetDevice(ctx->device));
  const size_t sn = static_cast<size_t>(n);
  const size_t plane = (sn + 3) & ~size_t(3);
  DevBuf<uint32_t> raw;
  if (aos_on_device && copy_aside && n > 0) {
    PCP_HIP_TRY(ctx, raw.ensure(static_cast<size_t>(n) * static_cast<size_t>(stride) / 4 + 4));
    PCP_HIP_TRY(ctx, hipMemcpyAsync(raw.p, aos, static_cast<size_t>(n) * static_cast<size_t>(stride), hipMemcpyDeviceToDevice, ctx->stream));
    aos = raw.p;
  }
  PCP_HIP_TRY(ctx, ctx->xyz.ensure(3 * plane + 4));
  PCP_HIP_TRY(ctx, ctx->sxyz.ensure(3 * plane + 4));
  PCP_HIP_TRY(ctx, ctx->perm.ensure(sn + 4));
  ctx->n = n;
  ctx->nonfinite_points = 0;
  ctx->sor_distances_live = false;
  ctx->sor_partial_slab = ctx->sor_partial_slabs = -1;
  ctx->n_tiles = 0;
  ctx->tile_order_live = false;
  ctx->have_intensity = false;
  ctx->nid_chunks = 0;
  ctx->colour_state_live = false;
  ctx->colour_result_live = false;
  ctx->labels_live = false;
  match_table_release(ctx);
  normals_release(ctx);
  ctx->crack->release();
  ctx->mls_count = 0;
  ctx->mls_result_live = false;
  end_smoothing_streams(ctx);
  ctx->css_ball = 0.0;
  std::fill(ctx->depth_valid.begin(), ctx->depth_valid.end(), uint8_t(0));
  ctx->hull_valid.clear();
  for (int a = 0; a < 3; ++a) ctx->host_min[a] = ctx->host_max[a] = 0.0f;
  if (n == 0) return PCP_OK;
  hipStream_t st = ctx->stream;
  float *dx = ctx->xyz.p, *dy = ctx->xyz.p + plane, *dz = ctx->xyz.p + 2 * plane;
  PCP_HIP_TRY(ctx, hipMemsetAsync(ctx->sxyz.p, 0, (3 * plane + 4) * 4, st));
  if (aos && aos_on_device) {
    hipLaunchKernelGGL(k_up_deinterleave, dim3(up_blocks(n)), dim3(kUpBlock), 0, st, static_cast<const uint32_t *>(aos), stride / 4, n,
                       dx, dy, dz);
  } else if (aos) {
    PCP_HIP_TRY(ctx, raw.ensure(static_cast<size_t>(n) * static_cast<size_t>(stride) / 4 + 4));
    PCP_HIP_TRY(ctx, hipMemcpyAsync(raw.p, aos, static_cast<size_t>(n) * static_cast<size_t>(stride), hipMemcpyHostToDevice, st));
    hipLaunchKernelGGL(k_up_deinterleave, dim3(up_blocks(n)), dim3(kUpBlock), 0, st, raw.p, stride / 4, n, dx, dy, dz);
  } else {
    PCP_HIP_TRY(ctx, hipMemcpyAsync(dx, x, sn * 4, hipMemcpyHostToDevice, st));
    PCP_HIP_TRY(ctx, hipMemcpyAsync(dy, y, sn * 4, hipMemcpyHostToDevice, st));
    PCP_HIP_TRY(ctx, hipMemcpyAsync(dz, z, sn * 4, hipMemcpyHostToDevice, st));
  }
  float mn[3], mx[3];
  unsigned long long nonfinite = 0;
  PCP_HIP_TRY(ctx, ctx->inv_perm.ensure(plane + 4));
  if (int rc = spatial_order(ctx, dx, dy, dz, n, ctx->perm.p, ctx->sxyz.p, ctx->sxyz.p + plane, ctx->sxyz.p + 2 * plane,
                             ctx->inv_perm.p, mn, mx, &nonfinite))
    return rc;
  raw.release();
  ctx->nonfinite_points = static_cast<int64_t>(nonfinite);
  for (int a = 0; a < 3; ++a) {
    ctx->host_min[a] = mn[a];
    ctx->host_max[a] = mx[a];
  }
  const int64_t tiles = (n + 63) / 64, groups = (tiles + 15) / 16;
  PCP_HIP_TRY(ctx, ctx->tile_sphere.ensure(static_cast<size_t>(tiles + groups) * 4 + 4));
  float4 *sph = reinterpret_cast<float4 *>(ctx->tile_sphere.p);
  hipLaunchKernelGGL(k_up_spheres<64>, dim3(static_cast<uint32_t>((tiles + 3) / 4)), dim3(kUpBlock), 0, st, ctx->sxyz.p,
                     ctx->sxyz.p + plane, ctx->sxyz.p + 2 * plane, n, sph, tiles);
  hipLaunchKernelGGL(k_up_spheres<1024>, dim3(static_cast<uint32_t>(groups)), dim3(kUpBlock), 0, st, ctx->sxyz.p,
                     ctx->sxyz.p + plane, ctx->sxyz.p + 2 * plane, n, sph + tiles, groups);
  PCP_HIP_TRY(ctx, hipGetLastError());
  ctx->n_tiles = tiles;
  PCP_HIP_TRY(ctx, hipStreamSynchronize(st));
  return PCP_OK;
}

}

using namespace pcp;

extern "C" {

int pcp_abi_version(void) { return PCP_ABI_VERSION; }

int pcp_create(int32_t device, pcp_context **out) {
  if (!out) {
    set_global_error("pcp_create: out is NULL");
    return PCP_ERR_INVALID;
  }
  *out = nullptr;
  int count = 0;
  hipError_t e = hipGetDeviceCount(&count);
  if (e != hipSuccess || count <= 0) {
    set_global_error("pcp_create: no HIP device available (%s); libpcp_hip has no CPU fallback",
                     e == hipSuccess ? "device count 0" : hipGetErrorString(e));
    return PCP_ERR_DEVICE;
  }
  if (device < 0 || device >= count) {
    set_global_error("pcp_create: device %d out of range (0..%d)", device, count - 1);
    return PCP_ERR_INVALID;
  }
  e = hipSetDevice(device);
  if (e == hipSuccess) {
    hipFuncAttributes a;
    const hipError_t pl[] = {hipFuncGetAttributes(&a, reinterpret_cast<const void *>(&k_up_bbox)), preload_colour(), preload_mls(), preload_grid(),
                             preload_nid(), preload_hpr(), preload_colour_smooth(), preload_match(),
                             preload_jpeg(), preload_stream_colour(), preload_ascii(), preload_ascii_parse(), preload_exposure(),
                             preload_voxel_reduce(), preload_normals(), preload_mask_edt(), preload_ortho(), preload_ortho_texture(), preload_facets(), preload_crack_width(), preload_crack_fuse(), preload_crack_length(), preload_crack_skeleton(), preload_image_balance()};
    for (hipError_t x : pl)
      if (x != hipSuccess && e == hipSuccess) e = x;
  }
  if (e != hipSuccess) {
    set_global_error("pcp_create: hipSetDevice(%d) / loading the gfx950 code objects failed: %s", device, hipGetErrorString(e));
    return PCP_ERR_DEVICE;
  }
  pcp_context *ctx = new (std::nothrow) pcp_context();
  if (ctx) ctx->crack.reset(new (std::nothrow) pcp::CrackMap());
  if (!ctx || !ctx->crack) {
    set_global_error("pcp_create: out of host memory");
    delete ctx;
    return PCP_ERR_NOMEM;
  }
  ctx->device = device;
  e = hipStreamCreateWithFlags(&ctx->own_stream, hipStreamNonBlocking);
  if (e != hipSuccess) {
    set_global_error("pcp_create: hipStreamCreate failed: %s", hipGetErrorString(e));
    delete ctx;
    return PCP_ERR_DEVICE;
  }
  ctx->stream = ctx->own_stream;
  {
    int prio_least = 0, prio_greatest = 0;
    e = hipDeviceGetStreamPriorityRange(&prio_least, &prio_greatest);
    if (e == hipSuccess) e = hipStreamCreateWithPriority(&ctx->copy_stream, hipStreamNonBlocking, prio_greatest);
  }
  for (int k = 0; k < 2 && e == hipSuccess; ++k) {
    e = hipEventCreateWithFlags(&ctx->result_ready[k], hipEventDisableTiming);
    if (e == hipSuccess) e = hipEventCreateWithFlags(&ctx->copy_done[k], hipEventDisableTiming);
  }
  if (e != hipSuccess) {
    set_global_error("pcp_create: copy stream / events: %s", hipGetErrorString(e));
    pcp_destroy(ctx);
    return PCP_ERR_DEVICE;
  }
  if (hipHostMalloc(&ctx->readback, pcp_context::kReadbackBytes, hipHostMallocDefault) != hipSuccess) {
    ctx->readback = nullptr;
    (void)hipGetLastError();
  }
  pcp_default_camera(&ctx->camera);
  pcp_default_cull_params(&ctx->cull);
  *out = ctx;
  return PCP_OK;
}

void pcp_destroy(pcp_context *ctx) {
  if (!ctx) return;
  (void)hipSetDevice(ctx->device);
  (void)hipStreamSynchronize(ctx->stream);
  if (ctx->copy_stream) (void)hipStreamSynchronize(ctx->copy_stream);
  for (hipStream_t us : ctx->upload_stream)
    if (us) {
      (void)hipStreamSynchronize(us);
      (void)hipStreamDestroy(us);
    }
  for (auto e : ctx->image_event)
    if (e) (void)hipEventDestroy(e);
  if (ctx->texels_idle) (void)hipEventDestroy(ctx->texels_idle);
  drain_timing(ctx);
  for (auto e : ctx->event_pool) (void)hipEventDestroy(e);
  ascii_parse_release(ctx);
  if (ctx->handoff) (void)hipEventDestroy(ctx->handoff);
  for (int k = 0; k < 2; ++k) {
    if (ctx->result_ready[k]) (void)hipEventDestroy(ctx->result_ready[k]);
    if (ctx->copy_done[k]) (void)hipEventDestroy(ctx->copy_done[k]);
  }
  if (ctx->copy_stream) (void)hipStreamDestroy(ctx->copy_stream);
  for (auto &lane : ctx->hpr_lane) lane.release();
  if (ctx->hpr_fork) (void)hipEventDestroy(ctx->hpr_fork);
  for (auto &e : ctx->hpr_join)
    if (e) (void)hipEventDestroy(e);
  if (ctx->readback) (void)hipHostFree(ctx->readback);
  if (ctx->own_stream) (void)hipStreamDestroy(ctx->own_stream);
  delete ctx;
}

const char *pcp_last_error(const pcp_context *ctx) { return ctx ? ctx->error.c_str() : g_error.c_str(); }

int pcp_set_stream(pcp_context *ctx, void *hip_stream) {
  if (!ctx) return PCP_ERR_INVALID;
  PCP_HIP_TRY(ctx, hipStreamSynchronize(ctx->stream));
  ctx->stream = hip_stream ? static_cast<hipStream_t>(hip_stream) : ctx->own_stream;
  return PCP_OK;
}

int pcp_synchronize(pcp_context *ctx) {
  if (!ctx) return PCP_ERR_INVALID;
  for (hipStream_t us : ctx->upload_stream)
    if (us) PCP_HIP_TRY(ctx, hipStreamSynchronize(us));
  std::fill(ctx->image_pending.begin(), ctx->image_pending.end(), uint8_t(0));
  PCP_HIP_TRY(ctx, hipStreamSynchronize(ctx->stream));
  PCP_HIP_TRY(ctx, hipStreamSynchronize(ctx->copy_stream));
  ctx->copy_pending[0] = ctx->copy_pending[1] = false;
  return PCP_OK;
}

void pcp_default_camera(pcp_camera *cam) {
  cam->fx = 4818.200388954926;
  cam->fy = 4819.10345841615;
  cam->cx = 2032.4178620390019;
  cam->cy = 1535.1895959282901;
  cam->k1 = 0.003043514741045163;
  cam->k2 = 0.06634739187544138;
  cam->p1 = -0.000217681797407554;
  cam->p2 = -0.0006654964142658197;
  cam->k3 = 0.0;
  cam->image_width = 4096;
  cam->image_height = 3000;
  cam->cull_width = 4096;
  cam->cull_height = 3000;
}

void pcp_default_cull_params(pcp_cull_params *p) {
  p->enable_depth_buffer_culling = 1;
// ... 276 lines not shown
```

### pointcloudprocessor_amd/csrc/pcp_internal.hpp

```cpp
#pragma once

#include <hip/hip_runtime.h>

#include <cstdarg>
#include <cstdint>
#include <chrono>
#include <cstdio>
#include <cstring>
#include <memory>
#include <string>
#include <type_traits>
#include <utility>
#include <vector>

#include "pcp_hip.h"

namespace pcp {

struct DevCamera {
  double fx, fy, cx, cy;
  double k1, k2, p1, p2, k3;
  double slack;
  float ds_f;
  double img_wd, img_hd;
// ... 144 lines not shown
  bool labels_fixed = false, with_label = false;
  pcp_ortho_frame frame{};
  int32_t fill_radius = 0;
  int64_t contributors = 0, atomics = 0, occupied = 0, filled = 0, adds = 0;
  DevBuf<unsigned long long> keys, scalars;
  DevBuf<uint32_t> payload;
  DevBuf<int32_t> source;
};

struct CrackMap;

struct Facets {
  bool live = false;
  int64_t rows = 0;
  DevBuf<int32_t> label, ids;
  DevBuf<long long> table;
  DevBuf<uint32_t> box;
  void release() {
    live = false;
    rows = 0;
    label.release(), ids.release(), table.release(), box.release();
  }
};

constexpr double kMaxGridCells = 536870912.0;
constexpr double kMaxSparseCells = 34359738368.0;
struct GridDesc {
  float minx, miny, minz, inv_cell;
  int32_t nx, ny, nz;
  int32_t reach;
  const unsigned long long *occ;
  const int32_t *occ_rank;
};

struct CloudView {
  const float *x, *y, *z;
  int64_t n;
  float mn[3], mx[3];
  const int32_t *remap;
};

struct VoxelDesc {
  float bminx, bminy, bminz, vs;
  int32_t NX, NY, NZ, it;
  int64_t words;
};

struct VgdStream {
  VoxelDesc v;
  GridDesc g;
  const int32_t *remap;
  size_t plane;
  int32_t order_poly;
  int32_t bricks;
  int32_t NBX, NBY, NBZ;
};
struct VgdChunk {
  int64_t word0, word1, voxels;
};

struct SmoothStream {
  pcp_mls_params p;
  VgdStream S;
  CloudView cv1;
  int64_t total_rows, kept_rows, rows_computed;
  double threshold, max_dx, min_margin;
  int32_t halo, redone;
  double sampled_dx;
  double seconds[4];
  double alloc_bytes;
};
struct ChainChunk {
  int64_t first_plane, last_plane, voxels, row0, rows;
};

enum class StreamPhase { None, Building, Open, Ended };
template <typename Stream, typename Chunk>
struct StreamState {
  StreamPhase phase = StreamPhase::None;
  Stream of{};
  std::vector<Chunk> chunks;
  int64_t next = 0;
  bool open() const { return phase == StreamPhase::Open; }
  bool idle() const { return phase == StreamPhase::None || phase == StreamPhase::Ended; }
  void end() {
    if (open()) phase = StreamPhase::Ended;
  }
};

}

struct pcp_context {
  int32_t device = 0;
  hipStream_t own_stream = nullptr;
  hipStream_t stream = nullptr;
  void *readback = nullptr;
  static constexpr size_t kReadbackBytes = 65536;
  mutable std::string error;

  bool have_camera = false;
  bool uv_tame = false;
  bool k3_dropped = false;
  pcp_camera camera{};
  pcp_cull_params cull{};
  pcp::DevCamera dcam{};

  int64_t n = 0;
  int64_t nonfinite_points = 0;
  pcp::DevBuf<float> xyz;
  pcp::DevBuf<float> sxyz;
  pcp::DevBuf<int32_t> perm;
  pcp::DevBuf<int32_t> inv_perm;
  std::vector<float> host_min = {0, 0, 0}, host_max = {0, 0, 0};

  int32_t n_frames = 0;
  std::vector<pcp_pose> poses;
  std::vector<pcp::DevFrame> hframes;
  pcp::DevBuf<pcp::DevFrame> frames;
  pcp::DevBuf<uint32_t> images;
  std::vector<uint8_t> image_set, mask_set;
  static constexpr int kUploadLanes = 2;
  hipStream_t upload_stream[kUploadLanes] = {nullptr, nullptr};
  pcp::DevBuf<uint8_t> upload_stage[kUploadLanes];
  pcp::DevBuf<uint8_t> jpeg_planes[kUploadLanes];
  std::vector<hipEvent_t> image_event;
  std::vector<uint8_t> image_pending;
  std::vector<uint8_t> image_lane;
  std::vector<uint64_t> image_seq;
  bool lane_must_wait[kUploadLanes] = {false, false};
  uint64_t upload_seq = 0;
  uint64_t upload_turn = 0;
  hipEvent_t texels_idle = nullptr;
  bool texels_touched = false;
  bool adjust_images = false;
  float saturation_scale = 1.0f, brightness_scale = 1.0f;
  pcp::DevBuf<int32_t> hsv_tables;
  pcp_balance_params balance{};
  uint8_t balance_gamma[256] = {};
  uint64_t balance_seq = 0;
  uint64_t balance_lane_seq[kUploadLanes] = {0, 0};
  pcp::DevBuf<uint32_t> balance_hist[kUploadLanes];
  pcp::DevBuf<uint8_t> balance_lut[kUploadLanes];
  pcp::DevBuf<uint32_t> balance_image;
  pcp::DevBuf<uint8_t> balance_bytes;

  pcp::DevBuf<uint32_t> depth;
  pcp::DevBuf<unsigned long long> depth_sq;
  std::vector<uint8_t> depth_valid;
  bool depth_from_batch = false;
  pcp::DevBuf<uint32_t> depth_accum;
  bool depth_accum_live = false;

  int64_t n_tiles = 0;
  pcp::DevBuf<float> tile_sphere;
  pcp::DevBuf<uint32_t> tile_mask, group_mask;
  pcp::DevBuf<uint32_t> tile_inside;
  int32_t mask_words = 0;
  pcp::DevBuf<int32_t> tile_work, tile_order, work_hist;
  bool tile_order_live = false;

  pcp::DevBuf<float> top_score;
  pcp::DevBuf<uint32_t> top_rgb;
  pcp::DevBuf<int32_t> top_frame;
  pcp::DevBuf<int32_t> view_count;
  pcp::DevBuf<uint32_t> rgba2[2];
  int32_t rgba_cur = 0;
  hipStream_t copy_stream = nullptr;
  hipEvent_t result_ready[2] = {nullptr, nullptr}, copy_done[2] = {nullptr, nullptr};
  bool copy_pending[2] = {false, false};
  bool colour_state_live = false;
  bool colour_result_live = false;
  bool label_fusion = false;
  bool labels_live = false;
  pcp::DevBuf<uint32_t> labels;
  bool gains_set = false;
  pcp::DevBuf<float> gains_dev;
  pcp::DevBuf<unsigned long long> pair_stats;
  int64_t pair_counters[5] = {0, 0, 0, 0, 0};
  bool pair_counters_live = false;

  pcp::VoxelReduce voxel_reduce;
  pcp::OrthoMap ortho;

  bool gn_live = false;
  float gn_radius = 0.0f;
  pcp::DevBuf<float> gn_normal;
  pcp::DevBuf<int32_t> gn_count;
  pcp::DevBuf<unsigned long long> gm_keys;
  pcp::DevBuf<uint32_t> gm_out;
  pcp::Facets facets;

  pcp::DevBuf<unsigned long long> md_bits;
  pcp::DevBuf<uint32_t> md_col, md_d2;
  pcp::DevBuf<int32_t> md_nearest;

  pcp::DevBuf<unsigned long long> cw_sat;
  pcp::DevBuf<uint8_t> cw_flags;
  pcp::DevBuf<int32_t> cw_i32;
  pcp::DevBuf<float> cw_f32;
  pcp::DevBuf<long long> cw_moments;

  std::unique_ptr<pcp::CrackMap> crack;

  bool match_live = false;
  double match_e = 0.0, match_rc = 0.0;
  float match_e2 = 0.0f;
  int64_t match_a = 0;
  int64_t match_entries = 0;
  pcp::DevBuf<uint8_t> match_in_a;
  pcp::DevBuf<int32_t> match_list;
  pcp::DevBuf<int64_t> match_off;
  pcp::DevBuf<int32_t> match_cols;
  pcp::DevBuf<unsigned long long> match_moved;

  pcp::DevBuf<int32_t> s_cell, s_pixel;
  pcp::DevBuf<float> s_range, s_cam;
  pcp::DevBuf<uint8_t> s_keep;
  pcp::DevBuf<uint32_t> s_u32;
  pcp::DevBuf<unsigned long long> s_counter;
  pcp::DevBuf<int32_t> s_tiles;

  static constexpr int kHprMaxLanes = 8;
  pcp::HprLane hpr_lane[kHprMaxLanes];
  int32_t hpr_last_lane = 0;
  hipEvent_t hpr_fork = nullptr, hpr_join[kHprMaxLanes] = {};
  pcp::DevBuf<uint32_t> hull_bits;
  std::vector<uint8_t> hull_valid;
  int64_t hpr_stats[10] = {0, 0, 0, 0, 0, 0, 0, 0, 0, 0};
  bool hpr_stats_pending = false;

  pcp::DevBuf<int32_t> g_cell, g_rank, g_start, g_order;
  pcp::DevBuf<unsigned long long> g_occ;
  pcp::DevBuf<int32_t> g_occ_rank;
  pcp::DevBuf<float> g_xyz;
  pcp::DevBuf<float> m_tmp;
  pcp::DevBuf<float> s_dist;
  pcp::DevBuf<double> m_state;
  double slp_radius = 0.05, slp_step = 0.01;
  pcp::DevBuf<float> slp_table;
  double slp_table_of[2] = {0.0, 0.0};
  pcp::DevBuf<int32_t> c_perm;
  pcp::DevBuf<uint8_t> m_flag;
  pcp::DevBuf<double> m_sums;
  pcp::DevBuf<int32_t> c_index;
  int32_t sor_partial_slab = -1, sor_partial_slabs = -1;
  bool sor_distances_live = false;
  pcp::DevBuf<uint8_t> c_mark;
  pcp::DevBuf<int32_t> c_where;
  pcp::DevBuf<float> c_xyz, c_xyz2;
  pcp::DevBuf<uint32_t> v_bitmap;
  pcp::DevBuf<int32_t> v_offsets;
  pcp::DevBuf<uint32_t> v_occ;
  pcp::DevBuf<int32_t> v_rank;
  pcp::DevBuf<unsigned long long> v_plane;
  pcp::DevBuf<int64_t> v_vox;
  pcp::DevBuf<float> mls_xyz, mls_normal, mls_curv;
  pcp::DevBuf<int32_t> mls_index;
  pcp::DevBuf<float> mls_alt_xyz, mls_alt_normal, mls_alt_curv;
  pcp::DevBuf<int32_t> mls_alt_index;
  int64_t mls_count = 0;
  bool mls_result_live = false;
  hipEvent_t handoff = nullptr;
  pcp::DevBuf<uint8_t> cc_out;
  pcp::DevBuf<uint8_t> ascii_in, ascii_len, ascii_text;
  pcp::DevBuf<unsigned long long> ascii_tiles;
  pcp::AsciiParseSlot parse_slot[2];
  hipStream_t parse_up = nullptr, parse_down = nullptr;
  pcp::StreamState<pcp::VgdStream, pcp::VgdChunk> emission;
  pcp::StreamState<pcp::SmoothStream, pcp::ChainChunk> chain;
  pcp::DevBuf<float> css_dist;
  pcp::DevBuf<float> s_kth;
  pcp::DevBuf<uint32_t> css_words;
  double css_ball = 0.0;
  double sor_redo_fraction = 0.0;

  pcp::DevBuf<float> intensity;
  bool have_intensity = false;
  pcp::DevBuf<float> nid_pts;
  pcp::DevBuf<int32_t> nid_chunk_kf;
  pcp::DevBuf<double> nid_hist;
  int64_t nid_chunks = 0, nid_points = 0;
  int32_t nid_frames = 0;
  int32_t nid_hist_bins = 0;

  bool timing = false;
  pcp::TimingSlot slots[PCP_K_COUNT];
  std::vector<pcp::PendingEvent> pending;
  std::vector<hipEvent_t> event_pool;
};

namespace pcp {

__device__ __forceinline__ int32_t cell_rank(const GridDesc &g, int64_t c) {
  const unsigned long long bits = g.occ[c >> 6];
  return g.occ_rank[c >> 6] + static_cast<int32_t>(__popcll(bits & ((1ull << (c & 63)) - 1ull)));
}

__device__ __forceinline__ int32_t cell_start(const GridDesc &g, const int32_t *__restrict__ start, int32_t zz, int32_t yy,
                                              int32_t xx) {
  if (!g.occ) return start[(zz * g.ny + yy) * g.nx + xx];
  return start[cell_rank(g, (static_cast<int64_t>(zz) * g.ny + yy) * g.nx + xx)];
}

__device__ __forceinline__ void grid_coords(const GridDesc &g, float x, float y, float z, int32_t &ix, int32_t &iy,
                                            int32_t &iz) {
  ix = min(max(static_cast<int32_t>(floorf((x - g.minx) * g.inv_cell)), 0), g.nx - 1);
  iy = min(max(static_cast<int32_t>(floorf((y - g.miny) * g.inv_cell)), 0), g.ny - 1);
// ... 136 lines not shown
```

### pointcloudprocessor_amd/csrc/pcp_tile_classify.hpp

```cpp
#pragma once

#include "pcp_device.hpp"

namespace pcp {

struct Interval {
  double lo, hi;
};
__device__ __forceinline__ Interval iv_add(Interval a, Interval b) { return {a.lo + b.lo, a.hi + b.hi}; }
__device__ __forceinline__ Interval iv_scale(double k, Interval a) {
  return k >= 0.0 ? Interval{k * a.lo, k * a.hi} : Interval{k * a.hi, k * a.lo};
}
__device__ __forceinline__ Interval iv_mul(Interval a, Interval b) {
  const double p0 = a.lo * b.lo, p1 = a.lo * b.hi, p2 = a.hi * b.lo, p3 = a.hi * b.hi;
  return {fmin(fmin(p0, p1), fmin(p2, p3)), fmax(fmax(p0, p1), fmax(p2, p3))};
}
__device__ __forceinline__ Interval iv_sqr(Interval a) {
  const double l = fabs(a.lo), h = fabs(a.hi);
  const double mx = fmax(l, h), mn = (a.lo <= 0.0 && a.hi >= 0.0) ? 0.0 : fmin(l, h);
  return {mn * mn, mx * mx};
}
__device__ __forceinline__ Interval iv_mul_pos(Interval a, Interval b) { return {a.lo * b.lo, a.hi * b.hi}; }
__device__ __forceinline__ Interval iv_mul_by_pos(Interval a, Interval b) {
  return {a.lo * (a.lo >= 0.0 ? b.lo : b.hi), a.hi * (a.hi >= 0.0 ? b.hi : b.lo)};
}
__device__ __forceinline__ double iv_rcp_pos(double b) {
  double r = __builtin_amdgcn_rcp(b);
  r = fma(fma(-b, r, 1.0), r, r);
  r = fma(fma(-b, r, 1.0), r, r);
  return r;
}
__device__ __forceinline__ Interval iv_pad(Interval a) {
  const double e = 1e-12 * (fabs(a.lo) + fabs(a.hi)) + 1e-300;
  return {a.lo - e, a.hi + e};
}

__device__ __forceinline__ int tile_classify(const DevCamera &c, const DevFrame &fr, float4 sph) {
  const double cx = sph.x, cy = sph.y, cz = sph.z;
  const float *m = fr.w2c;
  const double X = (m[0] * cx + m[1] * cy) + (m[2] * cz + m[3]);
  const double Y = (m[4] * cx + m[5] * cy) + (m[6] * cz + m[7]);
  const double Z = (m[8] * cx + m[9] * cy) + (m[10] * cz + m[11]);
  const double mag = fr.norm_bound * (fabs(cx) + fabs(cy) + fabs(cz) + 3.0 * sph.w) + fabs(static_cast<double>(m[3])) +
                     fabs(static_cast<double>(m[7])) + fabs(static_cast<double>(m[11])) + 1e-3;
  const double rho = fr.norm_bound * static_cast<double>(sph.w) * (1.0 + 1e-6) + 1e-6 * mag;
  if (!(rho >= 0.0) || !isfinite(X + Y + Z + rho)) return 0;
  if (Z + rho <= 0.0) return 1;
  if (Z - rho <= 0.0) return 0;
  const Interval zi{Z - rho, Z + rho};
  if (!(zi.lo >= 1e-290)) return 0;
  const Interval iz{iv_rcp_pos(zi.hi) * (1.0 - 1e-13), iv_rcp_pos(zi.lo) * (1.0 + 1e-13)};
  const Interval xn = iv_pad(iv_mul_by_pos(Interval{X - rho, X + rho}, iz));
  const Interval yn = iv_pad(iv_mul_by_pos(Interval{Y - rho, Y + rho}, iz));
  const Interval x2 = iv_sqr(xn), y2 = iv_sqr(yn);
  const Interval r2 = iv_add(x2, y2);
  const Interval r4 = iv_mul_pos(r2, r2);
  const Interval r6 = iv_mul_pos(r2, r4);
  Interval rc = iv_add(iv_add(iv_scale(c.k1, r2), iv_scale(c.k2, r4)), iv_scale(c.k3, r6));
  rc.lo += 1.0;
  rc.hi += 1.0;
  const Interval t1 = iv_scale(2.0, iv_mul(xn, yn));
  const Interval t2 = iv_add(r2, iv_scale(2.0, x2));
  const Interval t3 = iv_add(r2, iv_scale(2.0, y2));
  const Interval xd = iv_pad(iv_add(iv_add(iv_mul(rc, xn), iv_scale(c.p1, t1)), iv_scale(c.p2, t2)));
  const Interval yd = iv_pad(iv_add(iv_add(iv_mul(rc, yn), iv_scale(c.p1, t3)), iv_scale(c.p2, t1)));
  Interval u = iv_pad(iv_scale(c.fx, xd)), v = iv_pad(iv_scale(c.fy, yd));
  u.lo += c.cx; u.hi += c.cx;
  v.lo += c.cy; v.hi += c.cy;
  if (!isfinite(u.lo + u.hi + v.lo + v.hi)) return 0;
  if (u.hi < static_cast<double>(c.u_lo) || u.lo > static_cast<double>(c.u_hi) ||
      v.hi < static_cast<double>(c.v_lo) || v.lo > static_cast<double>(c.v_hi))
    return 1;
  return (u.lo > static_cast<double>(c.u_lo) + 1.0 && u.hi < static_cast<double>(c.u_hi) - 1.0 &&
          v.lo > static_cast<double>(c.v_lo) + 1.0 && v.hi < static_cast<double>(c.v_hi) - 1.0)
             ? 2
             : 0;
}

}
```

### pointcloudprocessor_amd/host_build.py

```python
from __future__ import annotations

import os
import subprocess

from . import _build

HOST = os.path.join(os.path.dirname(os.path.abspath(__file__)), "host")
BIN = os.path.join(HOST, "bin")
ROCM = os.environ.get("ROCM_PATH", "/opt/rocm")

TARGETS = {
    "pcp_shim_selftest": ["shim_selftest.cpp"],
    "PointCloudProcessor": ["main.cpp"],
    "image_dump": ["image_dump.cpp"],
    "format_selftest": ["format_selftest.cpp"],
    "parse_selftest": ["parse_selftest.cpp"],
    "visit_forms_selftest": ["visit_forms_selftest.cpp"],
    "k3_term_selftest": ["k3_term_selftest.cpp"],
    "voxel_reduce_selftest": ["voxel_reduce_selftest.cpp"],
    "normals_selftest": ["normals_selftest.cpp"],
    "ortho_selftest": ["ortho_selftest.cpp"],
    "ortho_texture_selftest": ["ortho_texture_selftest.cpp"],
    "crack_width_selftest": ["crack_width_selftest.cpp"],
    "crack_fuse_selftest": ["crack_fuse_selftest.cpp"],
    "crack_length_selftest": ["crack_length_selftest.cpp"],
    "crack_skeleton_selftest": ["crack_skeleton_selftest.cpp"],
    "image_balance_selftest": ["image_balance_selftest.cpp"],
    "facets_selftest": ["facets_selftest.cpp"],
}


def build(force: bool = False) -> dict:
    os.makedirs(BIN, exist_ok=True)
    out = {}
    for name, srcs in TARGETS.items():
        exe = os.path.join(BIN, name)
        deps = [os.path.join(HOST, s) for s in srcs] + [os.path.join(HOST, "pcp_shim.hpp"), os.path.join(HOST, "pcp_multi.hpp"), os.path.join(HOST, "pcd_io.hpp"), os.path.join(HOST, "image_io.hpp"), os.path.join(HOST, "pcd_device_reader.hpp"),
                                                       os.path.join(_build.CSRC, "pcp_ascii_parse.hpp"), os.path.join(_build.CSRC, "pcp_ascii.hpp"), os.path.join(_build.CSRC, "pcp_visit_forms.hpp"), os.path.join(_build.CSRC, "pcp_voxel_reduce.hpp"), os.path.join(_build.CSRC, "pcp_normals.hpp"), os.path.join(_build.CSRC, "pcp_ortho.hpp"), os.path.join(_build.CSRC, "pcp_ortho_texture.hpp"), os.path.join(_build.CSRC, "pcp_crack_width.hpp"), os.path.join(_build.CSRC, "pcp_crack_fuse.hpp"), os.path.join(_build.CSRC, "pcp_crack_length.hpp"), os.path.join(_build.CSRC, "pcp_crack_skeleton.hpp"), os.path.join(_build.CSRC, "pcp_image_balance.hpp"), os.path.join(_build.CSRC, "pcp_hsv.hpp"), os.path.join(_build.CSRC, "pcp_facets.hpp"), os.path.join(_build.CSRC, "pcp_eigen33_host.hpp"),
                                                       os.path.join(_build.INCLUDE, "pcp_hip.h")]
        deps = [d for d in deps if os.path.exists(d)]
        stale = force or not os.path.exists(exe) or any(os.path.getmtime(d) > os.path.getmtime(exe) for d in deps)
        if stale:
            extra = os.environ.get("PCP_HOST_CXXFLAGS", "").split()
            multi = ["-D__HIP_PLATFORM_AMD__", "-isystem", os.path.join(ROCM, "include")] if name == "PointCloudProcessor" else []
            multi_libs = ["-L", os.path.join(ROCM, "lib"), "-lrccl", "-lamdhip64", "-Wl,-rpath," + os.path.join(ROCM, "lib")] \
                if name == "PointCloudProcessor" else []
            cmd = ["g++", "-std=c++17", "-O2", "-ffp-contract=off", "-pthread", "-Wall", "-Wextra"] + extra + multi + ["-I", _build.INCLUDE, "-I", HOST] + [
                os.path.join(HOST, s) for s in srcs] + ["-L", _build.LIB_DIR, "-lpcp_hip"] + multi_libs + [
                                                        "-lz", "-Wl,-rpath,$ORIGIN/../../lib", "-o", exe]
            proc = subprocess.run(cmd, capture_output=True, text=True)
            if proc.returncode != 0:
                raise RuntimeError(f"g++ failed for {name}:\n{proc.stderr[-3000:]}")
        out[name] = exe
    return out
```

Before: 2.081 million.

## Cull tiles with per-axis box extents alongside bounding spheres

Tile and group bounds now carry per-axis half-extents next to the bounding sphere, and the frustum classification uses the tighter box-projected radius per camera row, capped by the sphere radius. The goal is to reject or wholly-accept more tile/frame pairs so fewer points are walked during colourisation. In exchange the bounds buffer doubles in size, the classify routine does a little more arithmetic per call, and the upload kernel does extra reductions. Debug accessors for the cloud order and the tile bounds are added, along with an offline simulation script.

```diff
diff --git a/include/pcp_hip.h b/include/pcp_hip.h
--- a/include/pcp_hip.h
+++ b/include/pcp_hip.h
@@ -378,6 +378,8 @@
 const char *pcp_kernel_name(int32_t kernel_id);
 int pcp_tile_mask_density(pcp_context *ctx, double *kept_fraction);
 int pcp_tile_masks(pcp_context *ctx, int64_t *tiles, int32_t *mask_words, uint32_t *out_words);
+int pcp_cloud_order(pcp_context *ctx, int32_t *out_perm);
+int pcp_tile_bounds(pcp_context *ctx, int64_t *tiles, float *out8);
 int pcp_sor_redo_fraction(pcp_context *ctx, double *fraction);
 int pcp_sor_distances(pcp_context *ctx, int64_t capacity, float *out_distance);
 int pcp_selftest_arithmetic(pcp_context *ctx, int64_t samples, uint64_t seed, int64_t *mismatches_fp64,
diff --git a/pointcloudprocessor_amd/_build.py b/pointcloudprocessor_amd/_build.py
--- a/pointcloudprocessor_amd/_build.py
+++ b/pointcloudprocessor_amd/_build.py
@@ -12,7 +12,7 @@
 
 SOURCES = ["pcp_context.hip", "pcp_colour.hip", "pcp_mls.hip", "pcp_grid.hip", "pcp_nid.hip", "pcp_hpr.hip", "pcp_colour_smooth.hip", "pcp_match.hip", "pcp_jpeg.hip",
            "pcp_stream_colour.hip", "pcp_ascii.hip", "pcp_ascii_parse.hip", "pcp_exposure.hip", "pcp_voxel_reduce.hip", "pcp_normals.hip", "pcp_mask_edt.hip", "pcp_ortho.hip", "pcp_ortho_texture.hip", "pcp_facets.hip", "pcp_crack_width.hip", "pcp_crack_fuse.hip", "pcp_crack_length.hip", "pcp_crack_skeleton.hip", "pcp_image_balance.hip"]
-HEADERS = ["pcp_internal.hpp", "pcp_device.hpp", "pcp_scan.hpp", "pcp_hsv.hpp", "pcp_exact.hpp", "pcp_ascii.hpp", "pcp_ascii_parse.hpp", "pcp_visit_forms.hpp", "pcp_voxel_reduce.hpp", "pcp_eigen33.hpp", "pcp_eigen33_host.hpp", "pcp_facets.hpp", "pcp_normals.hpp", "pcp_mask_edt.hpp", "pcp_ortho.hpp", "pcp_ortho_texture.hpp", "pcp_tile_classify.hpp", "pcp_crack_width.hpp", "pcp_crack_fuse.hpp", "pcp_crack_length.hpp", "pcp_crack_skeleton.hpp", "pcp_crack_map.hpp", "pcp_image_balance.hpp"]
+HEADERS = ["pcp_internal.hpp", "pcp_device.hpp", "pcp_scan.hpp", "pcp_hsv.hpp", "pcp_exact.hpp", "pcp_ascii.hpp", "pcp_ascii_parse.hpp", "pcp_visit_forms.hpp", "pcp_voxel_reduce.hpp", "pcp_eigen33.hpp", "pcp_eigen33_host.hpp", "pcp_facets.hpp", "pcp_normals.hpp", "pcp_mask_edt.hpp", "pcp_ortho.hpp", "pcp_ortho_texture.hpp", "pcp_tile_classify.hpp", "pcp_tile_box.hpp", "pcp_crack_width.hpp", "pcp_crack_fuse.hpp", "pcp_crack_length.hpp", "pcp_crack_skeleton.hpp", "pcp_crack_map.hpp", "pcp_image_balance.hpp"]
 
 HIPCC_FLAGS = [
     "--offload-arch=gfx950",
diff --git a/pointcloudprocessor_amd/capi.py b/pointcloudprocessor_amd/capi.py
--- a/pointcloudprocessor_amd/capi.py
+++ b/pointcloudprocessor_amd/capi.py
@@ -1570,5 +1570,18 @@
         self._check(self.lib.pcp_tile_masks(self.h, None, None, _ptr(out)))
         return out
 
+    def cloud_order(self) -> np.ndarray:
+        out = np.empty(int(self.lib.pcp_cloud_size(self.h)), np.int32)
+        self._check(self.lib.pcp_cloud_order(self.h, _ptr(out)))
+        return out
+
+    def tile_bounds(self) -> tuple[np.ndarray, np.ndarray]:
+        t = C.c_int64()
+        self._check(self.lib.pcp_tile_bounds(self.h, C.byref(t), None))
+        groups = (t.value + 15) // 16
+        out = np.empty((t.value + groups, 8), np.float32)
+        self._check(self.lib.pcp_tile_bounds(self.h, None, _ptr(out)))
+        return out[:t.value], out[t.value:]
+
     def kernel_name(self, kernel_id: int) -> str:
         return self.lib.pcp_kernel_name(C.c_int32(kernel_id)).decode()
diff --git a/pointcloudprocessor_amd/csrc/pcp_colour.hip b/pointcloudprocessor_amd/csrc/pcp_colour.hip
--- a/pointcloudprocessor_amd/csrc/pcp_colour.hip
+++ b/pointcloudprocessor_amd/csrc/pcp_colour.hip
@@ -102,7 +102,7 @@
 
 constexpr int kTileGroup = 16;
 
-__global__ __launch_bounds__(kBlock) void k_group_mask_flat(const float4 *__restrict__ spheres, int64_t groups, DevCamera cam,
+__global__ __launch_bounds__(kBlock) void k_group_mask_flat(const float4 *__restrict__ bounds, int64_t groups, DevCamera cam,
                                                             const DevFrame *__restrict__ frames, int32_t n_frames,
                                                             int32_t w0, int32_t w1, int32_t words,
                                                             uint32_t *__restrict__ group_mask,
@@ -119,7 +119,7 @@
   const int32_t w = w0 + static_cast<int32_t>(gw - group * nw);
   const int32_t f = (w << 5) + static_cast<int32_t>(idx & 31);
   int cls = 1;
-  if (live && f < n_frames) cls = cull_enabled ? tile_classify(cam, frames[f], spheres[group]) : 0;
+  if (live && f < n_frames) cls = cull_enabled ? tile_classify_box(cam, frames[f], bounds[2 * group], bounds[2 * group + 1]) : 0;
   const unsigned long long m = __ballot(cls != 1), in = __ballot(cls == 2);
   if (live && (idx & 31) == 0) {
     group_mask[group * words + w] = static_cast<uint32_t>((threadIdx.x & 32) ? (m >> 32) : m);
@@ -128,7 +128,7 @@
 }
 
 template <bool kInside>
-__global__ __launch_bounds__(kBlock) void k_tile_mask_dense(const float4 *__restrict__ spheres, int64_t tiles,
+__global__ __launch_bounds__(kBlock) void k_tile_mask_dense(const float4 *__restrict__ bounds, int64_t tiles,
                                                             DevCamera cam, const DevFrame *__restrict__ frames,
                                                             int32_t n_frames, int32_t w0, int32_t w1, int32_t words,
                                                             const uint32_t *__restrict__ group_mask,
@@ -152,7 +152,8 @@
   uint32_t word = whole;
   [[maybe_unused]] uint32_t inside = whole;
   if (todo) {
-    const float4 sph = spheres[have ? tile : tiles - 1];
+    const int64_t bt = have ? tile : tiles - 1;
+    const float4 sph = bounds[2 * bt], ext = bounds[2 * bt + 1];
     while (todo) {
       int32_t bit[4];
 #pragma unroll
@@ -162,7 +163,7 @@
       }
       const int32_t b = slot == 0 ? bit[0] : slot == 1 ? bit[1] : slot == 2 ? bit[2] : bit[3];
       int cls = 1;
-      if (b >= 0 && have) cls = cull_enabled ? tile_classify(cam, frames[(w << 5) + b], sph) : 0;
+      if (b >= 0 && have) cls = cull_enabled ? tile_classify_box(cam, frames[(w << 5) + b], sph, ext) : 0;
       const unsigned long long keep = __ballot(cls != 1);
       [[maybe_unused]] unsigned long long ins = 0ull;
       if constexpr (kInside) ins = __ballot(cls == 2);
@@ -1746,18 +1747,18 @@
     {
       LaunchTimer t(ctx, PCP_K_TILE_MASK);
       const int64_t groups = div_up(ctx->n_tiles, kTileGroup);
-      const float4 *tile_sph = reinterpret_cast<const float4 *>(ctx->tile_sphere.p);
+      const float4 *tile_bnd = reinterpret_cast<const float4 *>(ctx->tile_bounds.p);
       const size_t gwords = static_cast<size_t>(groups) * ctx->mask_words;
       PCP_HIP_TRY(ctx, ctx->group_mask.ensure(2 * gwords + 8));
       uint32_t *group_inside = ctx->group_mask.p + gwords + 4;
       hipLaunchKernelGGL(k_group_mask_flat, dim3(std::max(blocks_for(groups * (w1 - w0) * 32), blocks_for(2 * kWorkBins))),
-                         dim3(kBlock), 0, ctx->stream, tile_sph + ctx->n_tiles, groups, ctx->dcam, ctx->frames.p, ctx->n_frames,
+                         dim3(kBlock), 0, ctx->stream, tile_bnd + 2 * ctx->n_tiles, groups, ctx->dcam, ctx->frames.p, ctx->n_frames,
                          w0, w1, ctx->mask_words, ctx->group_mask.p, group_inside, cull_tiles ? 1 : 0, ctx->work_hist.p,
                          2 * kWorkBins, z_maps ? reinterpret_cast<unsigned long long *>(ctx->depth_sq.p) : nullptr,
                          z_maps ? map_cells : int64_t(0));
       uint32_t *tile_inside = is_common_camera(ctx) ? nullptr : ctx->tile_inside.p;
       hipLaunchKernelGGL(tile_inside ? k_tile_mask_dense<true> : k_tile_mask_dense<false>, dim3(static_cast<uint32_t>(div_up(groups * (w1 - w0), kBlock / 64))), dim3(kBlock),
-                         0, ctx->stream, tile_sph, ctx->n_tiles, ctx->dcam, ctx->frames.p, ctx->n_frames, w0, w1,
+                         0, ctx->stream, tile_bnd, ctx->n_tiles, ctx->dcam, ctx->frames.p, ctx->n_frames, w0, w1,
                          ctx->mask_words, ctx->group_mask.p, group_inside, ctx->tile_mask.p, tile_inside, cull_tiles ? 1 : 0);
       if ((rc = sort_tiles_by_work(ctx, w0, w1, ctx->tile_order.p)) != PCP_OK) return rc;
       ctx->tile_order_live = true;
@@ -2187,6 +2188,28 @@
   return PCP_OK;
 }
 
+int pcp_cloud_order(pcp_context *ctx, int32_t *out_perm) {
+  if (!ctx || !out_perm) return PCP_ERR_INVALID;
+  if (ctx->n == 0) return set_error(ctx, PCP_ERR_STATE, "pcp_cloud_order: no cloud (call pcp_upload_cloud)");
+  PCP_HIP_TRY(ctx, hipMemcpyAsync(out_perm, ctx->perm.p, static_cast<size_t>(ctx->n) * 4, hipMemcpyDeviceToHost, ctx->stream));
+  PCP_HIP_TRY(ctx, hipStreamSynchronize(ctx->stream));
+  return PCP_OK;
+}
+
+int pcp_tile_bounds(pcp_context *ctx, int64_t *tiles, float *out8) {
+  if (!ctx) return PCP_ERR_INVALID;
+  if (ctx->n == 0 || ctx->n_tiles == 0 || !ctx->tile_bounds.p)
+    return set_error(ctx, PCP_ERR_STATE, "pcp_tile_bounds: no cloud (call pcp_upload_cloud)");
+  if (tiles) *tiles = ctx->n_tiles;
+  if (out8) {
+    const int64_t groups = div_up(ctx->n_tiles, kTileGroup);
+    PCP_HIP_TRY(ctx, hipMemcpyAsync(out8, ctx->tile_bounds.p, static_cast<size_t>(ctx->n_tiles + groups) * 8 * 4, hipMemcpyDeviceToHost,
+                                    ctx->stream));
+    PCP_HIP_TRY(ctx, hipStreamSynchronize(ctx->stream));
+  }
+  return PCP_OK;
+}
+
 int pcp_colour_result_device(pcp_context *ctx, void **device_ptr, int64_t *n_words) {
   if (!ctx) return PCP_ERR_INVALID;
   if (!ctx->colour_result_live)
diff --git a/pointcloudprocessor_amd/csrc/pcp_context.hip b/pointcloudprocessor_amd/csrc/pcp_context.hip
--- a/pointcloudprocessor_amd/csrc/pcp_context.hip
+++ b/pointcloudprocessor_amd/csrc/pcp_context.hip
@@ -298,13 +298,13 @@
 }
 
 template <int kSpan>
-__global__ __launch_bounds__(kUpBlock) void k_up_spheres(const float *__restrict__ sx, const float *__restrict__ sy,
+__global__ __launch_bounds__(kUpBlock) void k_up_bounds(const float *__restrict__ sx, const float *__restrict__ sy,
                                                         const float *__restrict__ sz, int64_t n,
                                                         float4 *__restrict__ out, int64_t count) {
   constexpr int kLanes = kSpan >= kUpBlock ? kUpBlock : kSpan;
   constexpr int kPer = kSpan / kLanes;
   constexpr int kSpheresPerBlock = kUpBlock / kLanes;
-  __shared__ double red[7][kUpBlock / 64];
+  __shared__ double red[10][kUpBlock / 64];
   const int sub = threadIdx.x / kLanes, l = threadIdx.x % kLanes;
   const int64_t sphere = static_cast<int64_t>(blockIdx.x) * kSpheresPerBlock + sub;
   const int64_t b = sphere * kSpan;
@@ -347,7 +347,7 @@
   float c[3];
 #pragma unroll
   for (int a = 0; a < 3; ++a) c[a] = static_cast<float>(0.5 * (lo[a] + hi[a]));
-  double r2 = 0.0;
+  double r2 = 0.0, h[3] = {0.0, 0.0, 0.0};
 #pragma unroll
   for (int q = 0; q < kPer; ++q)
     if (have[q]) {
@@ -355,17 +355,33 @@
       const double dy = static_cast<double>(py[q]) - static_cast<double>(c[1]);
       const double dz = static_cast<double>(pz[q]) - static_cast<double>(c[2]);
       r2 = fmax(r2, (dx * dx + dy * dy) + dz * dz);
-    }
-  for (int o = (kLanes < 64 ? kLanes : 64) / 2; o >= 1; o >>= 1) r2 = fmax(r2, __shfl_xor(r2, o, 64));
+      h[0] = fmax(h[0], fabs(dx));
+      h[1] = fmax(h[1], fabs(dy));
+      h[2] = fmax(h[2], fabs(dz));
+    }
+  for (int o = (kLanes < 64 ? kLanes : 64) / 2; o >= 1; o >>= 1) {
+    r2 = fmax(r2, __shfl_xor(r2, o, 64));
+#pragma unroll
+    for (int a = 0; a < 3; ++a) h[a] = fmax(h[a], __shfl_xor(h[a], o, 64));
+  }
   if (kLanes > 64) {
-    if ((threadIdx.x & 63) == 0) red[6][threadIdx.x >> 6] = r2;
+    if ((threadIdx.x & 63) == 0) {
+      red[6][threadIdx.x >> 6] = r2;
+      for (int a = 0; a < 3; ++a) red[7 + a][threadIdx.x >> 6] = h[a];
+    }
     __syncthreads();
-    for (int k = 0; k < kUpBlock / 64; ++k) r2 = fmax(r2, red[6][k]);
+    for (int k = 0; k < kUpBlock / 64; ++k) {
+      r2 = fmax(r2, red[6][k]);
+      for (int a = 0; a < 3; ++a) h[a] = fmax(h[a], red[7 + a][k]);
+    }
   }
   if (l == 0 && sphere < count) {
-    float r = static_cast<float>(sqrt(r2) * (1.0 + 1e-6));
-    r = isfinite(r) ? __uint_as_float(__float_as_uint(r) + 1u) : r;
-    out[sphere] = make_float4(c[0], c[1], c[2], r);
+    const auto up = [](double v) {
+      const float r = static_cast<float>(v * (1.0 + 1e-6));
+      return isfinite(r) ? __uint_as_float(__float_as_uint(r) + 1u) : r;
+    };
+    out[2 * sphere] = make_float4(c[0], c[1], c[2], up(sqrt(r2)));
+    out[2 * sphere + 1] = make_float4(up(h[0]), up(h[1]), up(h[2]), 0.0f);
   }
 }
 
@@ -507,12 +523,12 @@
     ctx->host_max[a] = mx[a];
   }
   const int64_t tiles = (n + 63) / 64, groups = (tiles + 15) / 16;
-  PCP_HIP_TRY(ctx, ctx->tile_sphere.ensure(static_cast<size_t>(tiles + groups) * 4 + 4));
-  float4 *sph = reinterpret_cast<float4 *>(ctx->tile_sphere.p);
-  hipLaunchKernelGGL(k_up_spheres<64>, dim3(static_cast<uint32_t>((tiles + 3) / 4)), dim3(kUpBlock), 0, st, ctx->sxyz.p,
+  PCP_HIP_TRY(ctx, ctx->tile_bounds.ensure(static_cast<size_t>(tiles + groups) * 8 + 4));
+  float4 *sph = reinterpret_cast<float4 *>(ctx->tile_bounds.p);
+  hipLaunchKernelGGL(k_up_bounds<64>, dim3(static_cast<uint32_t>((tiles + 3) / 4)), dim3(kUpBlock), 0, st, ctx->sxyz.p,
                      ctx->sxyz.p + plane, ctx->sxyz.p + 2 * plane, n, sph, tiles);
-  hipLaunchKernelGGL(k_up_spheres<1024>, dim3(static_cast<uint32_t>(groups)), dim3(kUpBlock), 0, st, ctx->sxyz.p,
-                     ctx->sxyz.p + plane, ctx->sxyz.p + 2 * plane, n, sph + tiles, groups);
+  hipLaunchKernelGGL(k_up_bounds<1024>, dim3(static_cast<uint32_t>(groups)), dim3(kUpBlock), 0, st, ctx->sxyz.p,
+                     ctx->sxyz.p + plane, ctx->sxyz.p + 2 * plane, n, sph + 2 * tiles, groups);
   PCP_HIP_TRY(ctx, hipGetLastError());
   ctx->n_tiles = tiles;
   PCP_HIP_TRY(ctx, hipStreamSynchronize(st));
diff --git a/pointcloudprocessor_amd/csrc/pcp_internal.hpp b/pointcloudprocessor_amd/csrc/pcp_internal.hpp
--- a/pointcloudprocessor_amd/csrc/pcp_internal.hpp
+++ b/pointcloudprocessor_amd/csrc/pcp_internal.hpp
@@ -320,7 +320,7 @@
   bool depth_accum_live = false;
 
   int64_t n_tiles = 0;
-  pcp::DevBuf<float> tile_sphere;
+  pcp::DevBuf<float> tile_bounds;
   pcp::DevBuf<uint32_t> tile_mask, group_mask;
   pcp::DevBuf<uint32_t> tile_inside;
   int32_t mask_words = 0;
diff --git a/pointcloudprocessor_amd/csrc/pcp_tile_box.hpp b/pointcloudprocessor_amd/csrc/pcp_tile_box.hpp
--- /dev/null
+++ b/pointcloudprocessor_amd/csrc/pcp_tile_box.hpp
@@ -0,0 +1,33 @@
+#pragma once
+
+#if defined(__HIPCC__)
+#include <hip/hip_runtime.h>
+#define PCP_TB_HD __host__ __device__ __forceinline__
+#else
+#include <cmath>
+#define PCP_TB_HD inline
+#endif
+
+namespace pcp {
+
+struct TileInflation {
+  double sphere;
+  double row[3];
+};
+
+PCP_TB_HD TileInflation tile_inflation(const float *m, double s, double cx, double cy, double cz, double r, double hx, double hy,
+                                       double hz) {
+  const double mag = s * (fabs(cx) + fabs(cy) + fabs(cz) + 3.0 * r) + fabs(static_cast<double>(m[3])) +
+                     fabs(static_cast<double>(m[7])) + fabs(static_cast<double>(m[11])) + 1e-3;
+  const double slack = 1e-6 * mag;
+  TileInflation t;
+  t.sphere = s * r * (1.0 + 1e-6) + slack;
+  for (int k = 0; k < 3; ++k) {
+    const double box = (fabs(static_cast<double>(m[4 * k])) * hx + fabs(static_cast<double>(m[4 * k + 1])) * hy) +
+                       fabs(static_cast<double>(m[4 * k + 2])) * hz;
+    t.row[k] = fmin(t.sphere, box * (1.0 + 1e-6) + slack);
+  }
+  return t;
+}
+
+}
diff --git a/pointcloudprocessor_amd/csrc/pcp_tile_classify.hpp b/pointcloudprocessor_amd/csrc/pcp_tile_classify.hpp
--- a/pointcloudprocessor_amd/csrc/pcp_tile_classify.hpp
+++ b/pointcloudprocessor_amd/csrc/pcp_tile_classify.hpp
@@ -1,6 +1,7 @@
 #pragma once
 
 #include "pcp_device.hpp"
+#include "pcp_tile_box.hpp"
 
 namespace pcp {
 
@@ -77,4 +78,45 @@
              : 0;
 }
 
+__device__ __forceinline__ int tile_classify_box(const DevCamera &c, const DevFrame &fr, float4 sph, float4 ext) {
+  const double cx = sph.x, cy = sph.y, cz = sph.z;
+  const float *m = fr.w2c;
+  const double X = (m[0] * cx + m[1] * cy) + (m[2] * cz + m[3]);
+  const double Y = (m[4] * cx + m[5] * cy) + (m[6] * cz + m[7]);
+  const double Z = (m[8] * cx + m[9] * cy) + (m[10] * cz + m[11]);
+  const TileInflation inf = tile_inflation(m, fr.norm_bound, cx, cy, cz, sph.w, ext.x, ext.y, ext.z);
+  const double rho = inf.sphere, rx = inf.row[0], ry = inf.row[1], rz = inf.row[2];
+  if (!(rho >= 0.0) || !isfinite(X + Y + Z + rho)) return 0;
+  if (Z + rz <= 0.0) return 1;
+  if (Z - rz <= 0.0) return 0;
+  const Interval zi{Z - rz, Z + rz};
+  if (!(zi.lo >= 1e-290)) return 0;
+  const Interval iz{iv_rcp_pos(zi.hi) * (1.0 - 1e-13), iv_rcp_pos(zi.lo) * (1.0 + 1e-13)};
+  const Interval xn = iv_pad(iv_mul_by_pos(Interval{X - rx, X + rx}, iz));
+  const Interval yn = iv_pad(iv_mul_by_pos(Interval{Y - ry, Y + ry}, iz));
+  const Interval x2 = iv_sqr(xn), y2 = iv_sqr(yn);
+  const Interval r2 = iv_add(x2, y2);
+  const Interval r4 = iv_mul_pos(r2, r2);
+  const Interval r6 = iv_mul_pos(r2, r4);
+  Interval rc = iv_add(iv_add(iv_scale(c.k1, r2), iv_scale(c.k2, r4)), iv_scale(c.k3, r6));
+  rc.lo += 1.0;
+  rc.hi += 1.0;
+  const Interval t1 = iv_scale(2.0, iv_mul(xn, yn));
+  const Interval t2 = iv_add(r2, iv_scale(2.0, x2));
+  const Interval t3 = iv_add(r2, iv_scale(2.0, y2));
+  const Interval xd = iv_pad(iv_add(iv_add(iv_mul(rc, xn), iv_scale(c.p1, t1)), iv_scale(c.p2, t2)));
+  const Interval yd = iv_pad(iv_add(iv_add(iv_mul(rc, yn), iv_scale(c.p1, t3)), iv_scale(c.p2, t1)));
+  Interval u = iv_pad(iv_scale(c.fx, xd)), v = iv_pad(iv_scale(c.fy, yd));
+  u.lo += c.cx; u.hi += c.cx;
+  v.lo += c.cy; v.hi += c.cy;
+  if (!isfinite(u.lo + u.hi + v.lo + v.hi)) return 0;
+  if (u.hi < static_cast<double>(c.u_lo) || u.lo > static_cast<double>(c.u_hi) ||
+      v.hi < static_cast<double>(c.v_lo) || v.lo > static_cast<double>(c.v_hi))
+    return 1;
+  return (u.lo > static_cast<double>(c.u_lo) + 1.0 && u.hi < static_cast<double>(c.u_hi) - 1.0 &&
+          v.lo > static_cast<double>(c.v_lo) + 1.0 && v.hi < static_cast<double>(c.v_hi) - 1.0)
+             ? 2
+             : 0;
 }
+
+}
diff --git a/pointcloudprocessor_amd/host/tile_bounds_selftest.cpp b/pointcloudprocessor_amd/host/tile_bounds_selftest.cpp
--- /dev/null
+++ b/pointcloudprocessor_amd/host/tile_bounds_selftest.cpp
@@ -0,0 +1,145 @@
+#include <algorithm>
+#include <cmath>
+#include <cstdint>
+#include <cstdio>
+#include <cstdlib>
+#include <cstring>
+#include <vector>
+
+#include "../csrc/pcp_tile_box.hpp"
+
+static uint64_t rng_state = 0x2545f4914f6cdd1dull;
+static uint64_t next_u64() {
+  rng_state += 0x9e3779b97f4a7c15ull;
+  uint64_t v = rng_state;
+  v = (v ^ (v >> 30)) * 0xbf58476d1ce4e5b9ull;
+  v = (v ^ (v >> 27)) * 0x94d049bb133111ebull;
+  return v ^ (v >> 31);
+}
+static double uniform(double lo, double hi) { return lo + (hi - lo) * (static_cast<double>(next_u64() >> 11) * 0x1p-53); }
+
+static float next_up(float v) {
+  if (!std::isfinite(v)) return v;
+  uint32_t b;
+  std::memcpy(&b, &v, 4);
+  b += 1u;
+  std::memcpy(&v, &b, 4);
+  return v;
+}
+static float inflate(double v) { return next_up(static_cast<float>(v * (1.0 + 1e-6))); }
+
+static double norm_bound(const float *m) {
+  double rowmax = 0.0;
+  for (int a = 0; a < 3; ++a) {
+    double row = 0.0;
+    for (int b = 0; b < 3; ++b) {
+      double g = 0.0;
+      for (int k = 0; k < 3; ++k) g += static_cast<double>(m[4 * k + a]) * static_cast<double>(m[4 * k + b]);
+      row += std::fabs(g);
+    }
+    rowmax = std::max(rowmax, row);
+  }
+  return std::sqrt(rowmax) * (1.0 + 1e-9);
+}
+
+static void rigid_matrix(float *m) {
+  double q[4], nrm = 0.0;
+  for (double &v : q) {
+    v = uniform(-1.0, 1.0);
+    nrm += v * v;
+  }
+  nrm = std::sqrt(nrm) + 1e-12;
+  for (double &v : q) v /= nrm;
+  const double w = q[0], x = q[1], y = q[2], z = q[3];
+  const double R[9] = {1 - 2 * (y * y + z * z), 2 * (x * y - w * z), 2 * (x * z + w * y), 2 * (x * y + w * z), 1 - 2 * (x * x + z * z),
+                       2 * (y * z - w * x), 2 * (x * z - w * y), 2 * (y * z + w * x), 1 - 2 * (x * x + y * y)};
+  for (int r = 0; r < 3; ++r) {
+    for (int c = 0; c < 3; ++c) m[4 * r + c] = static_cast<float>(R[3 * r + c]);
+    m[4 * r + 3] = static_cast<float>(uniform(-50.0, 50.0));
+  }
+}
+static void wild_matrix(float *m) {
+  for (int k = 0; k < 12; ++k) {
+    const double mag = std::ldexp(uniform(1.0, 2.0), static_cast<int>(next_u64() % 61) - 20);
+    m[k] = (next_u64() % 7 == 0) ? 0.0f : static_cast<float>((next_u64() & 1) ? mag : -mag);
+  }
+}
+
+int main(int argc, char **argv) {
+  const long tiles = argc > 1 ? std::atol(argv[1]) : 20000;
+  const int kInterior = 24, kMatrices = 6;
+  long outside = 0, points = 0, rows = 0, rows_box = 0, flat_rows = 0, flat_rows_box = 0;
+  std::vector<float> px, py, pz;
+  for (long t = 0; t < tiles; ++t) {
+    float lo[3], hi[3];
+    const bool flat = t % 3 == 0;
+    const int flat_axis = static_cast<int>(next_u64() % 3);
+    for (int a = 0; a < 3; ++a) {
+      const double c = uniform(-60.0, 60.0), w = std::ldexp(uniform(1.0, 2.0), static_cast<int>(next_u64() % 8) - 6);
+      lo[a] = static_cast<float>(c - w);
+      hi[a] = (flat && a == flat_axis) ? (t % 6 == 0 ? lo[a] : static_cast<float>(c - w + 1e-3 * w)) : static_cast<float>(c + w);
+      if (hi[a] < lo[a]) std::swap(lo[a], hi[a]);
+    }
+    px.clear(); py.clear(); pz.clear();
+    for (int k = 0; k < 8; ++k) {
+      px.push_back((k & 1) ? hi[0] : lo[0]);
+      py.push_back((k & 2) ? hi[1] : lo[1]);
+      pz.push_back((k & 4) ? hi[2] : lo[2]);
+    }
+    for (int k = 0; k < kInterior; ++k) {
+      px.push_back(std::min(hi[0], std::max(lo[0], static_cast<float>(uniform(lo[0], hi[0])))));
+      py.push_back(std::min(hi[1], std::max(lo[1], static_cast<float>(uniform(lo[1], hi[1])))));
+      pz.push_back(std::min(hi[2], std::max(lo[2], static_cast<float>(uniform(lo[2], hi[2])))));
+    }
+    const float c[3] = {static_cast<float>(0.5 * (static_cast<double>(lo[0]) + hi[0])), static_cast<float>(0.5 * (static_cast<double>(lo[1]) + hi[1])),
+                        static_cast<float>(0.5 * (static_cast<double>(lo[2]) + hi[2]))};
+    double r2 = 0.0, h[3] = {0.0, 0.0, 0.0};
+    for (size_t k = 0; k < px.size(); ++k) {
+      const double dx = static_cast<double>(px[k]) - c[0], dy = static_cast<double>(py[k]) - c[1], dz = static_cast<double>(pz[k]) - c[2];
+      r2 = std::fmax(r2, (dx * dx + dy * dy) + dz * dz);
+      h[0] = std::fmax(h[0], std::fabs(dx));
+      h[1] = std::fmax(h[1], std::fabs(dy));
+      h[2] = std::fmax(h[2], std::fabs(dz));
+    }
+    const float r = inflate(std::sqrt(r2)), hx = inflate(h[0]), hy = inflate(h[1]), hz = inflate(h[2]);
+    for (int mi = 0; mi < kMatrices; ++mi) {
+      float m[12];
+      if (mi < kMatrices / 2) rigid_matrix(m); else wild_matrix(m);
+      const double s = norm_bound(m);
+      const pcp::TileInflation inf = pcp::tile_inflation(m, s, c[0], c[1], c[2], r, hx, hy, hz);
+      const double cx = c[0], cy = c[1], cz = c[2];
+      const double C[3] = {(m[0] * cx + m[1] * cy) + (m[2] * cz + m[3]), (m[4] * cx + m[5] * cy) + (m[6] * cz + m[7]),
+                           (m[8] * cx + m[9] * cy) + (m[10] * cz + m[11])};
+      for (int k = 0; k < 3; ++k) {
+        if (!(inf.row[k] <= inf.sphere)) ++outside;
+        ++rows;
+        if (inf.row[k] < inf.sphere) ++rows_box;
+        if (flat && mi < kMatrices / 2) {
+          ++flat_rows;
+          if (inf.row[k] < inf.sphere) ++flat_rows_box;
+        }
+      }
+      for (size_t k = 0; k < px.size(); ++k) {
+        const float x = px[k], y = py[k], z = pz[k];
+        const float got[3] = {x * m[0] + (y * m[1] + (z * m[2] + m[3])), x * m[4] + (y * m[5] + (z * m[6] + m[7])),
+                              x * m[8] + (y * m[9] + (z * m[10] + m[11]))};
+        ++points;
+        for (int a = 0; a < 3; ++a) {
+          if (!std::isfinite(got[a])) continue;
+          if (!(std::fabs(static_cast<double>(got[a]) - C[a]) <= inf.row[a])) {
+            if (++outside <= 10)
+              std::printf("outside: tile %ld matrix %d point %zu axis %d: |%.17g - %.17g| > %.17g (sphere %.17g)\n", t, mi, k, a,
+                          static_cast<double>(got[a]), C[a], inf.row[a], inf.sphere);
+          }
+        }
+      }
+    }
+  }
+  std::printf("tile bounds: %ld tiles, %ld transformed points, %ld outside\n", tiles, points, outside);
+  std::printf("rows: %ld, the box's bound is the smaller in %ld; rigid matrices on flat boxes: %ld of %ld\n", rows, rows_box, flat_rows_box,
+              flat_rows);
+  const bool exercised = flat_rows_box * 2 > flat_rows;
+  if (!exercised) std::printf("the box's bound was hardly ever the smaller\n");
+  std::printf("tile_bounds_selftest: %ld outside\n", outside);
+  return outside == 0 && exercised ? 0 : 1;
+}
diff --git a/pointcloudprocessor_amd/host_build.py b/pointcloudprocessor_amd/host_build.py
--- a/pointcloudprocessor_amd/host_build.py
+++ b/pointcloudprocessor_amd/host_build.py
@@ -27,6 +27,7 @@
     "crack_skeleton_selftest": ["crack_skeleton_selftest.cpp"],
     "image_balance_selftest": ["image_balance_selftest.cpp"],
     "facets_selftest": ["facets_selftest.cpp"],
+    "tile_bounds_selftest": ["tile_bounds_selftest.cpp"],
 }
 
 
@@ -36,7 +37,7 @@
     for name, srcs in TARGETS.items():
         exe = os.path.join(BIN, name)
         deps = [os.path.join(HOST, s) for s in srcs] + [os.path.join(HOST, "pcp_shim.hpp"), os.path.join(HOST, "pcp_multi.hpp"), os.path.join(HOST, "pcd_io.hpp"), os.path.join(HOST, "image_io.hpp"), os.path.join(HOST, "pcd_device_reader.hpp"),
-                                                       os.path.join(_build.CSRC, "pcp_ascii_parse.hpp"), os.path.join(_build.CSRC, "pcp_ascii.hpp"), os.path.join(_build.CSRC, "pcp_visit_forms.hpp"), os.path.join(_build.CSRC, "pcp_voxel_reduce.hpp"), os.path.join(_build.CSRC, "pcp_normals.hpp"), os.path.join(_build.CSRC, "pcp_ortho.hpp"), os.path.join(_build.CSRC, "pcp_ortho_texture.hpp"), os.path.join(_build.CSRC, "pcp_crack_width.hpp"), os.path.join(_build.CSRC, "pcp_crack_fuse.hpp"), os.path.join(_build.CSRC, "pcp_crack_length.hpp"), os.path.join(_build.CSRC, "pcp_crack_skeleton.hpp"), os.path.join(_build.CSRC, "pcp_image_balance.hpp"), os.path.join(_build.CSRC, "pcp_hsv.hpp"), os.path.join(_build.CSRC, "pcp_facets.hpp"), os.path.join(_build.CSRC, "pcp_eigen33_host.hpp"),
+                                                       os.path.join(_build.CSRC, "pcp_ascii_parse.hpp"), os.path.join(_build.CSRC, "pcp_ascii.hpp"), os.path.join(_build.CSRC, "pcp_visit_forms.hpp"), os.path.join(_build.CSRC, "pcp_voxel_reduce.hpp"), os.path.join(_build.CSRC, "pcp_normals.hpp"), os.path.join(_build.CSRC, "pcp_ortho.hpp"), os.path.join(_build.CSRC, "pcp_ortho_texture.hpp"), os.path.join(_build.CSRC, "pcp_crack_width.hpp"), os.path.join(_build.CSRC, "pcp_crack_fuse.hpp"), os.path.join(_build.CSRC, "pcp_crack_length.hpp"), os.path.join(_build.CSRC, "pcp_crack_skeleton.hpp"), os.path.join(_build.CSRC, "pcp_image_balance.hpp"), os.path.join(_build.CSRC, "pcp_hsv.hpp"), os.path.join(_build.CSRC, "pcp_facets.hpp"), os.path.join(_build.CSRC, "pcp_eigen33_host.hpp"), os.path.join(_build.CSRC, "pcp_tile_box.hpp"),
                                                        os.path.join(_build.INCLUDE, "pcp_hip.h")]
         deps = [d for d in deps if os.path.exists(d)]
         stale = force or not os.path.exists(exe) or any(os.path.getmtime(d) > os.path.getmtime(exe) for d in deps)
diff --git a/profiles/tile_bounds_sim.py b/profiles/tile_bounds_sim.py
--- /dev/null
+++ b/profiles/tile_bounds_sim.py
@@ -0,0 +1,189 @@
+#!/usr/bin/env python3
+import os
+import sys
+import time
+
+import numpy as np
+
+sys.path.insert(0, os.path.dirname(os.path.dirname(os.path.abspath(__file__))))
+from oracle import np_oracle
+from pointcloudprocessor_amd import synth
+
+F_ALL = 256
+f64 = np.float64
+
+
+def hilbert30(ix, iy, iz):
+    X = [ix.astype(np.uint32).copy(), iy.astype(np.uint32).copy(), iz.astype(np.uint32).copy()]
+    Q = 512
+    while Q > 1:
+        P = np.uint32(Q - 1)
+        for i in range(3):
+            hit = (X[i] & np.uint32(Q)) != 0
+            t = np.where(hit, np.uint32(0), (X[0] ^ X[i]) & P)
+            X[0] = np.where(hit, X[0] ^ P, X[0] ^ t)
+            X[i] = X[i] ^ t if i else X[0]
+        Q >>= 1
+    X[1] ^= X[0]
+    X[2] ^= X[1]
+    t = np.zeros_like(X[0])
+    Q = 512
+    while Q > 1:
+        t = np.where((X[2] & np.uint32(Q)) != 0, t ^ np.uint32(Q - 1), t)
+        Q >>= 1
+    X = [a ^ t for a in X]
+
+    def spread(v):
+        v = v.astype(np.uint64) & np.uint64(0x3FF)
+        v = (v | (v << np.uint64(16))) & np.uint64(0x30000FF)
+        v = (v | (v << np.uint64(8))) & np.uint64(0x300F00F)
+        v = (v | (v << np.uint64(4))) & np.uint64(0x30C30C3)
+        v = (v | (v << np.uint64(2))) & np.uint64(0x9249249)
+        return v
+
+    return (spread(X[0]) << np.uint64(2)) | (spread(X[1]) << np.uint64(1)) | spread(X[2])
+
+
+def hilbert_order(p):
+    mn, mx = p.min(axis=0), p.max(axis=0)
+    sc = np.float32(1023.999) / (mx - mn)
+    cell = np.clip((p - mn) * sc, 0, 1023).astype(np.uint32)
+    return np.argsort(hilbert30(cell[:, 0], cell[:, 1], cell[:, 2]), kind="stable")
+
+
+def refine(p, block):
+    n = len(p)
+    order = np.arange(n)
+    seg = block
+    while seg > 64:
+        sid = np.arange(n) // seg
+        q = p[order]
+        starts = np.arange(0, n, seg)
+        ext = np.stack([np.maximum.reduceat(q[:, a], starts) - np.minimum.reduceat(q[:, a], starts) for a in range(3)], axis=1)
+        axis = np.argmax(ext, axis=1)[sid]
+        key = q[np.arange(n), axis]
+        order = order[np.lexsort((key, sid))]
+        seg //= 2
+    return order
+
+
+def bounds(p, span):
+    n = len(p)
+    cnt = (n + span - 1) // span
+    pad = cnt * span - n
+    q = np.concatenate([p, np.repeat(p[-1:], pad, axis=0)]).reshape(cnt, span, 3).astype(f64)
+    c = (0.5 * (q.min(axis=1) + q.max(axis=1))).astype(np.float32)
+    d = np.abs(q - c[:, None, :].astype(f64))
+    up = lambda v: np.nextafter((v * (1 + 1e-6)).astype(np.float32), np.float32(np.inf))
+    return c, up(np.sqrt((d * d).sum(axis=2).max(axis=1))), up(d.max(axis=1))
+
+
+def iv_mul(a, b):
+    ps = [a[0] * b[0], a[0] * b[1], a[1] * b[0], a[1] * b[1]]
+    return np.minimum.reduce(ps), np.maximum.reduce(ps)
+
+
+def iv_scale(k, a):
+    return (k * a[0], k * a[1]) if k >= 0 else (k * a[1], k * a[0])
+
+
+def iv_sqr(a):
+    l, h = np.abs(a[0]), np.abs(a[1])
+    mn = np.where((a[0] <= 0) & (a[1] >= 0), 0.0, np.minimum(l, h))
+    return mn * mn, np.maximum(l, h) ** 2
+
+
+def classify(cam, box, w2c, c, r, h):
+    M = np.asarray(w2c, np.float32).reshape(3, 4).astype(f64)
+    nb = np.sqrt(np.abs(M[:, :3].T @ M[:, :3]).sum(axis=1).max()) * (1 + 1e-9)
+    c, r = c.astype(f64), r.astype(f64)
+    C = c @ M[:, :3].T + M[:, 3]
+    mag = nb * (np.abs(c).sum(axis=1) + 3 * r) + np.abs(M[:, 3]).sum() + 1e-3
+    rho = nb * r * (1 + 1e-6) + 1e-6 * mag
+    R = np.repeat(rho[:, None], 3, axis=1)
+    if h is not None:
+        R = np.minimum(R, (h.astype(f64) @ np.abs(M[:, :3]).T) * (1 + 1e-6) + 1e-6 * mag[:, None])
+    X, Y, Z = C.T
+    out = np.zeros(len(c), np.int8)
+    out[Z + R[:, 2] <= 0] = 1
+    go = Z - R[:, 2] > 0
+    with np.errstate(all="ignore"):
+        iz = (1 / (Z + R[:, 2]), 1 / np.where(go, Z - R[:, 2], 1.0))
+        xn = iv_mul((X - R[:, 0], X + R[:, 0]), iz)
+        yn = iv_mul((Y - R[:, 1], Y + R[:, 1]), iz)
+        x2, y2 = iv_sqr(xn), iv_sqr(yn)
+        r2 = (x2[0] + y2[0], x2[1] + y2[1])
+        r4 = (r2[0] * r2[0], r2[1] * r2[1])
+        r6 = (r2[0] * r4[0], r2[1] * r4[1])
+        rc = [sum(t) for t in zip(iv_scale(cam["k1"], r2), iv_scale(cam["k2"], r4), iv_scale(cam["k3"], r6))]
+        rc = (rc[0] + 1, rc[1] + 1)
+        t1 = iv_scale(2.0, iv_mul(xn, yn))
+        t2 = (r2[0] + 2 * x2[0], r2[1] + 2 * x2[1])
+        t3 = (r2[0] + 2 * y2[0], r2[1] + 2 * y2[1])
+        xd = [sum(t) for t in zip(iv_mul(rc, xn), iv_scale(cam["p1"], t1), iv_scale(cam["p2"], t2))]
+        yd = [sum(t) for t in zip(iv_mul(rc, yn), iv_scale(cam["p1"], t3), iv_scale(cam["p2"], t1))]
+        u = [cam["fx"] * xd[0] + cam["cx"], cam["fx"] * xd[1] + cam["cx"]]
+        v = [cam["fy"] * yd[0] + cam["cy"], cam["fy"] * yd[1] + cam["cy"]]
+    u_lo, v_lo, u_hi, v_hi = box
+    miss = (u[1] < u_lo) | (u[0] > u_hi) | (v[1] < v_lo) | (v[0] > v_hi)
+    inside = (u[0] > u_lo + 1) & (u[1] < u_hi - 1) & (v[0] > v_lo + 1) & (v[1] < v_hi - 1)
+    out[go & miss] = 1
+    out[go & ~miss & inside] = 2
+    return out
+
+
+def main():
+    n = int(sys.argv[1]) if len(sys.argv) > 1 else 10_000_000
+    k = int(sys.argv[2]) if len(sys.argv) > 2 else 6
+    blocks = [int(b) for b in sys.argv[3].split(",")] if len(sys.argv) > 3 else [4096]
+    cam = synth.camera_dict("cfg")
+    ds = 14
+    mw, mh = cam["cull_width"] // ds, cam["cull_height"] // ds
+    box = (-(ds + 0.5), -(ds + 0.5), max(ds * mw, cam["image_width"]) + 0.5, max(ds * mh, cam["image_height"]) + 0.5)
+    x, y, z, _ = synth.make_cloud(n)
+    poses, _ = synth.make_trajectory(F_ALL)
+    frames = [round(i * (F_ALL - 1) / (k - 1)) for i in range(k)] if k > 1 else [0]
+    p_in = np.stack([x, y, z], axis=1)
+    t0 = time.time()
+    hil = hilbert_order(p_in)
+    p_h = p_in[hil]
+    print(f"# {n} points, keyframes {frames} scaled to {F_ALL}; Hilbert order in {time.time() - t0:.0f} s", flush=True)
+    w2cs = [np_oracle.pose_to_matrices(poses[f])[0] for f in frames]
+    cand = []
+    for w2c in w2cs:
+        pf = np_oracle.project_frame(cam, w2c, x, y, z)
+        cand.append(((pf["cell"] >= 0) & (pf["pixel"] >= 0))[hil])
+    scale = F_ALL / len(frames) / 1e6
+    print("| order | bounds | mean tile radius, half-extents (cm) | group pairs kept | wholly inside | tile classifications | walked | with a candidate | candidates lost |")
+    print("|---|---|---|---|---|---|---|---|---|")
+    orders = [("Hilbert", np.arange(n))] + [(f"refined, blocks of {b}", refine(p_h, b)) for b in blocks]
+    for name, order in orders:
+        p = p_h[order]
+        tc, tr, th = bounds(p, 64)
+        gc, gr, gh = bounds(p, 1024)
+        n_tiles = len(tc)
+        tile_group = np.arange(n_tiles) // 16
+        cand_tile = []
+        for cf in cand:
+            ct = np.zeros(n_tiles, bool)
+            ct[np.nonzero(cf[order])[0] // 64] = True
+            cand_tile.append(ct)
+        he = np.sort(th.astype(f64), axis=1)[:, ::-1].mean(axis=0) * 100
+        for bname, use_h in (("spheres", False), ("boxes", True)):
+            tot = np.zeros(6)
+            for w2c, ct in zip(w2cs, cand_tile):
+                g = classify(cam, box, w2c, gc, gr, gh if use_h else None)
+                t_need = (g == 0)[tile_group]
+                t = np.ones(n_tiles, np.int8)
+                idx = np.nonzero(t_need)[0]
+                t[idx] = classify(cam, box, w2c, tc[idx], tr[idx], th[idx] if use_h else None)
+                t[(g == 2)[tile_group]] = 2
+                walked = t != 1
+                tot += [(g != 1).sum(), (g == 2).sum(), len(idx), walked.sum(), ct.sum(), (ct & ~walked).sum()]
+            m = tot * scale
+            print(f"| {name} | {bname} | {tr.astype(f64).mean() * 100:.2f}; {he[0]:.1f} x {he[1]:.1f} x {he[2]:.1f} | {m[0]:.3f} | {m[1]:.3f} | {m[2]:.2f} | {m[3]:.3f} | {m[4]:.3f} | {int(tot[5])} |",
+                  flush=True)
+
+
+if __name__ == "__main__":
+    main()
```

Result: faster. 2.114 million, median of 6 (+1.6%).
